# Nobita421/signature-Gan

Measured on AMD Instinct MI355X. Metric: signature images/sec (G+D train step, bs64 64x64 z=100), higher is better.
Workload: dtype f32; 1 GPU; configs[1]: reference conv G/D 64x64x1, z=100, batch 64 per GPU, f32, n_critic=1; global_batch=64, parallelism=dp1

## Files before the change

### include/siggan.h

```cpp
#ifndef SIGGAN_H
#define SIGGAN_H

#include <stddef.h>
#include <stdint.h>

#ifdef __cplusplus
extern "C" {
#endif

#define SIGGAN_ABI_VERSION 4

enum {
    SIGGAN_OK = 0,
    SIGGAN_E_INVALID = -1,
    SIGGAN_E_STATE = -2,
    SIGGAN_E_HIP = -3,
    SIGGAN_E_NOMEM = -4
};

typedef struct siggan_ctx siggan_ctx;

typedef struct siggan_config {
    int32_t device;
    int32_t latent_dim;
    int32_t image_size;
    int32_t image_channels;
    int32_t max_batch;
    float   dropout;
    float   leaky_slope;
    uint64_t seed;
    int32_t dtype;
    float   f16_grad_scale;
    int32_t spectral_norm;
    float   g_leaky_slope;
} siggan_config;
enum { SIGGAN_DTYPE_F32 = 0, SIGGAN_DTYPE_BF16 = 1, SIGGAN_DTYPE_F16 = 2 };

typedef struct siggan_storage {
    float *g_params, *g_grads, *g_exp_avg, *g_exp_avg_sq, *g_adam_steps;
    float *g_bn_running_mean, *g_bn_running_var;
    int64_t *g_bn_batches;
    float *d_params, *d_grads, *d_exp_avg, *d_exp_avg_sq, *d_adam_steps;
    float *d_sn_u, *d_sn_v;
} siggan_storage;

typedef struct siggan_hyper {
    double lr, beta1, beta2, eps;
    float label_smoothing;
    float clip_max_norm;
    float grad_scale;
} siggan_hyper;

enum {
    SIGGAN_M_D_LOSS = 0, SIGGAN_M_D_LOSS_REAL, SIGGAN_M_D_LOSS_FAKE, SIGGAN_M_D_REAL_MEAN,
    SIGGAN_M_D_FAKE_MEAN, SIGGAN_M_D_REAL_ACC, SIGGAN_M_D_FAKE_ACC, SIGGAN_M_D_GRAD_NORM,
    SIGGAN_M_G_LOSS, SIGGAN_M_G_FAKE_MEAN, SIGGAN_M_G_GRAD_NORM,
    SIGGAN_M_D_SKIPPED, SIGGAN_M_G_SKIPPED,
    SIGGAN_M_COUNT = 16
};

int siggan_abi_version(void);
const char *siggan_last_error(void);
int siggan_create(const siggan_config *cfg, siggan_ctx **out);
int siggan_destroy(siggan_ctx *ctx);

int64_t siggan_param_count(const siggan_ctx *ctx, int which);
int32_t siggan_param_tensors(const siggan_ctx *ctx, int which);
int siggan_param_span(const siggan_ctx *ctx, int which, int32_t idx, int64_t *offset, int64_t *numel);
int64_t siggan_bn_count(const siggan_ctx *ctx);
int64_t siggan_sn_count(const siggan_ctx *ctx, int which);
int32_t siggan_bn_layers(const siggan_ctx *ctx);
int64_t siggan_workspace_bytes(const siggan_ctx *ctx);

int siggan_bind(siggan_ctx *ctx, const siggan_storage *st);
int siggan_params_changed(siggan_ctx *ctx);
int siggan_seed(siggan_ctx *ctx, uint64_t seed, uint64_t offset);
int siggan_rng_state(siggan_ctx *ctx, uint64_t *seed, uint64_t *offset);
#define SIGGAN_MODE_GRAPH 1
#define SIGGAN_MODE_OVERLAP 2
int siggan_set_mode(siggan_ctx *ctx, int32_t mode);

enum { SIGGAN_STEP_TRAINER = 0, SIGGAN_STEP_ABLATION = 1 };
int siggan_set_step_variant(siggan_ctx *ctx, int32_t variant);

int siggan_g_forward(siggan_ctx *ctx, const float *z_dev, int32_t batch, int32_t training,
                     float *images_dev, void *stream);

enum { SIGGAN_IS_NEG = 0, SIGGAN_IS_INK_SIGNED = 1, SIGGAN_IS_INK_UNIT = 2, SIGGAN_IS_COUNT = 3 };
int siggan_g_generate_u8(siggan_ctx *ctx, const float *z_dev, int32_t batch, uint8_t *u8_dev,
                         float *images_dev, int32_t *stats_dev, float threshold, void *stream);

int siggan_d_forward(siggan_ctx *ctx, const float *x_dev, int32_t batch, int32_t training,
                     const float *masks_dev, float *probs_dev, float *features_dev, void *stream);

int siggan_d_step(siggan_ctx *ctx, const float *real_dev, int32_t batch, const float *z_dev,
                  const float *masks_dev, const siggan_hyper *hp, float *metrics_dev,
                  float *metrics_host, void *stream);
int siggan_g_step(siggan_ctx *ctx, int32_t batch, const float *z_dev, const siggan_hyper *hp,
                  float *metrics_dev, float *metrics_host, void *stream);

#define SIGGAN_COMM_ID_BYTES 128
int siggan_comm_unique_id(void *id_out);
int siggan_comm_init(siggan_ctx *ctx, int32_t rank, int32_t world, const void *id);
int siggan_comm_destroy(siggan_ctx *ctx);
int32_t siggan_comm_world(const siggan_ctx *ctx);
int siggan_comm_broadcast(siggan_ctx *ctx, void *buf_dev, int64_t bytes, int32_t root, void *stream);

int siggan_d_grads(siggan_ctx *ctx, const float *real_dev, int32_t batch, const float *z_dev,
                   const float *masks_dev, const siggan_hyper *hp, float *metrics_dev, void *stream);
int siggan_step_begin(siggan_ctx *ctx, const float *real_dev, int32_t batch, const float *z_dev,
                      const float *masks_dev, const float *zg_dev, const siggan_hyper *hp,
                      float *metrics_dev, void *stream);
int siggan_stage_real(siggan_ctx *ctx, const float *real_dev, int32_t batch, void *stream);
int siggan_d_apply(siggan_ctx *ctx, const siggan_hyper *hp, float *metrics_dev, float *metrics_host,
                   void *stream);
int siggan_g_grads(siggan_ctx *ctx, int32_t batch, const float *z_dev, const siggan_hyper *hp,
                   float *metrics_dev, void *stream);
int siggan_g_apply(siggan_ctx *ctx, const siggan_hyper *hp, float *metrics_dev, float *metrics_host,
                   void *stream);

int siggan_op_conv4x4s2(siggan_ctx *ctx, int32_t form, const void *in_dev, const float *w_dev,
                        void *out_dev, int32_t batch, int32_t h_in, int32_t c_in, int32_t c_out,
                        void *stream);
int siggan_op_conv4x4s2_wgrad(siggan_ctx *ctx, const void *small_dev, const void *large_dev,
                              float *dw_dev, int32_t batch, int32_t h_small, int32_t c_small,
                              int32_t c_large, void *stream);
int siggan_op_adam(siggan_ctx *ctx, float *p_dev, float *g_dev, float *m_dev, float *v_dev,
                   int64_t n, int32_t step, const siggan_hyper *hp, void *stream);
int siggan_op_randn(siggan_ctx *ctx, float *out_dev, int64_t n, void *stream);
int siggan_augment_batch(int32_t device, const uint8_t *cache_dev, int64_t n_images, const int32_t *index_dev,
                         const int32_t *params_dev, const int16_t *tables_dev, const float *lut_dev,
                         float *out_dev, int32_t batch, int32_t size, int32_t augment, int32_t fill,
                         void *stream);
int siggan_image_stats(int32_t device, const float *x_dev, int32_t batch, int64_t pixels,
                       float threshold, int32_t *stats_dev, void *stream);
int siggan_device_info(int32_t device, int32_t *compute_units, int32_t *clock_khz, int64_t *hbm_bytes);
int siggan_prof_enable(siggan_ctx *ctx, int32_t on);
int32_t siggan_prof_slots(void);
int siggan_prof_read(siggan_ctx *ctx, int32_t idx, char *name, int32_t name_cap, int64_t *launches,
                     double *ms, double *flops, double *bytes);
int siggan_prof_launch(siggan_ctx *ctx, int64_t idx, int32_t *fields, int32_t n, int64_t *count);

int siggan_debug_tensor(siggan_ctx *ctx, const char *name, int32_t index, float *out_dev, int64_t n, void *stream);

#ifdef __cplusplus
}
#endif
#endif
```

### signature-gan_amd/csrc/gconv.h

```cpp
#pragma once
#include <hip/hip_runtime.h>
#include <stdint.h>
#include <vector>

#include "act.h"

namespace siggan {

enum Epilogue : int {
    EPI_RAW = 0,
    EPI_BIAS_LRELU_DROP,
    EPI_AFFINE_RELU,
    EPI_LRELU_BWD,
    EPI_BN_BWD_STATS,
};

struct GConvArgs {
    int dt;
    const void* in;
    const void* wp;
    void* out;
    int B, Hi, Wi, Ci, Co;
    int lgHr, lgWr;
    int Ho, Wo;
    int form;
    int M;
    int epi;
    const float* bias;
    const float* noise;
    const float* scale;
    const float* shift;
    const void* aref;
    const float* bnp;
    float* stat0;
    float* stat1;
    int64_t stat_cap;
    const float* cls_w;
    float* cls_part;
    float slope;
    float gslope;
    float* slab;
    int64_t slab_floats;
    size_t slab_stride;
    const float* zeros;
};

struct BnBwdParams { f32x4 sc, sf, mu, rs; };
__device__ __forceinline__ BnBwdParams bn_bwd_params(const float* __restrict__ bnp, int Co, int co) {
    BnBwdParams q;
    q.sc = *reinterpret_cast<const f32x4*>(bnp + co); q.sf = *reinterpret_cast<const f32x4*>(bnp + Co + co);
    q.mu = *reinterpret_cast<const f32x4*>(bnp + 2 * Co + co); q.rs = *reinterpret_cast<const f32x4*>(bnp + 3 * Co + co);
    return q;
}
template <class T, bool LK>
__device__ __forceinline__ void bn_bwd_stat_terms(const f32x4 v, const f32x4 y, const BnBwdParams& q, float gs, f32x4& s0, f32x4& s1) {
#pragma unroll
    for (int e = 0; e < 4; ++e) {
        const float vq = (float)(T)v[e];
        const float d = g_dact<LK>(fmaf(y[e], q.sc[e], q.sf[e]), vq, gs);
        s0[e] += d;
        s1[e] = fmaf(d, (y[e] - q.mu[e]) * q.rs[e], s1[e]);
    }
}
__host__ __device__ inline bool gen_lk(const GConvArgs& a) {
    return a.gslope != 0.f && (a.epi == EPI_AFFINE_RELU || a.epi == EPI_BN_BWD_STATS);
}

struct WgradArgs {
    int dt;
    const void* S;
    const void* L;
    float* slab;
    float* dw;
    float* db;
    int B, Cs, Cl;
    int lgHs, lgWs, lgCl;
    int K;
    int kchunk;
    const float* zeros;
};

struct Prof {
    struct Rec {
        int id; double flops, bytes; hipEvent_t e0, e1;
        int form, epi_req, epi, M, Ci, Co;
    };
    static constexpr int NID = 8;
    std::vector<Rec> recs;
    static const char* name(int id);
    void begin(int id, double flops, double bytes, hipStream_t st);
    void shape(const GConvArgs& a, int epi_req);
    void clear();
};
extern Prof* g_prof;

int launch_gconv(const GConvArgs& a, hipStream_t st);
void launch_gconv16(int cfg, const GConvArgs& a, dim3 grid, hipStream_t st, hipEvent_t e0, hipEvent_t e1, int kq = 1);
void launch_wgrad16(bool small, const WgradArgs& a, dim3 grid, hipStream_t st, hipEvent_t e0, hipEvent_t e1);
int launch_wgrad(WgradArgs a, int max_splits, hipStream_t st);

}
```

### signature-gan_amd/csrc/gconv.hip

```cpp
#include "gconv.h"
#include <hip/hip_ext.h>

namespace siggan {


static constexpr int BK = 32;
static constexpr int PAD = 4;

__device__ __forceinline__ int xcd_remap(int bid, int nwg) {
    const int q = nwg >> 3, r = nwg & 7, xcd = bid & 7, idx = bid >> 3;
    return (xcd < r ? xcd * (q + 1) : r * (q + 1) + (xcd - r) * q) + idx;
}

template <int BM, int BN, int WM, int WN, int BK = 32, int DEEP = 0, int KQ = 1, bool LK = false>
__global__ __launch_bounds__(256 * KQ) void k_gconv(const GConvArgs a) {
    constexpr int TM = BM / (32 * WM), TN = BN / (32 * WN);
    constexpr int PA = BM / 32, PB = BN / 32;
    constexpr int KC = BK / 32;
    constexpr int LD = BK + 4;
    __shared__ __attribute__((aligned(16))) float smem[KQ * 2 * LD * (BM + BN)];
    const int quad = KQ > 1 ? (int)(threadIdx.x >> 8) : 0;
    float* const sA = smem + quad * (2 * LD * (BM + BN));
    float* const sB = sA + 2 * LD * BM;

    const int tid = threadIdx.x & 255, lane = tid & 63, wave = tid >> 6;
    const int li = lane & 31, lh = lane >> 5;
    const int wm = wave / WN, wn = wave % WN;
    const float* const a_in = static_cast<const float*>(a.in);
    const float* const a_wp = static_cast<const float*>(a.wp);

    const int tiles_n = a.Co / BN;
    const int bid = xcd_remap(blockIdx.x, gridDim.x);
    const int m0 = (bid / tiles_n) * BM, n0 = (bid % tiles_n) * BN;
    const int cls = blockIdx.z, ph = cls >> 1, pw = cls & 1;
    const int Hr = 1 << a.lgHr, Wr = 1 << a.lgWr;
    const int ntaps = a.form == 0 ? 16 : 4;
    const int Ktot = ntaps * a.Ci;
    const int lgcpt = 31 - __builtin_clz(a.Ci / BK);
    const int nk_all = ntaps << lgcpt;
    const int kper = (nk_all + gridDim.y * KQ - 1) / (gridDim.y * KQ);
    const int k_lo = (blockIdx.y * KQ + quad) * kper;
    const int k_hi = min(nk_all, k_lo + kper);
    const int nk = k_hi - k_lo;

    const int kc = tid & 7, rloc = tid >> 3;
    const float* a_base[PA];
    int a_ih0[PA], a_iw0[PA];
#pragma unroll
    for (int p = 0; p < PA; ++p) {
        const int m = m0 + rloc + 32 * p;
        if (m < a.M) {
            const int n = m >> (a.lgHr + a.lgWr);
            const int rh = (m >> a.lgWr) & (Hr - 1), rw = m & (Wr - 1);
            a_base[p] = a_in + (size_t)n * a.Hi * a.Wi * a.Ci + kc * 4;
            if (a.form == 0) { a_ih0[p] = 2 * rh - 1; a_iw0[p] = 2 * rw - 1; }
            else             { a_ih0[p] = rh + ph;    a_iw0[p] = rw + pw; }
        } else {
            a_base[p] = a_in; a_ih0[p] = -(1 << 20); a_iw0[p] = -(1 << 20);
        }
    }
    const float* wcur = a_wp + ((size_t)cls * a.Co + n0 + rloc) * Ktot + kc * 4 + (size_t)k_lo * BK;

    const float* a_cur[PA];
    int a_step[PA];
    int l_tap = k_lo >> lgcpt, l_cc = k_lo & ((1 << lgcpt) - 1);
    auto set_tap = [&]() __attribute__((always_inline)) {
        int dh, dw;
        if (a.form == 0) { dh = l_tap >> 2; dw = l_tap & 3; } else { dh = -(l_tap >> 1); dw = -(l_tap & 1); }
#pragma unroll
        for (int p = 0; p < PA; ++p) {
            const int ih = a_ih0[p] + dh, iw = a_iw0[p] + dw;
            const bool ok = (unsigned)ih < (unsigned)a.Hi && (unsigned)iw < (unsigned)a.Wi;
            a_cur[p] = ok ? a_base[p] + ((size_t)(ih * a.Wi + iw) * a.Ci + l_cc * BK) : a.zeros;
            a_step[p] = ok ? BK : 0;
        }
    };
    constexpr int NSET = DEEP ? 2 : 1;
    f32x4 ra[NSET][PA][KC], rb[NSET][PB][KC];
    auto load_tile = [&](int set = 0) __attribute__((always_inline)) {
#pragma unroll
        for (int p = 0; p < PA; ++p) {
#pragma unroll
            for (int q = 0; q < KC; ++q) ra[set][p][q] = *reinterpret_cast<const f32x4*>(a_cur[p] + 32 * q);
// ... 269 lines not shown
        for (int t = 0; t < 4; ++t)
            rb[t] = *reinterpret_cast<const f32x4*>(w_row + (size_t)cls * a.Co * Ktot + t * CI + cc * BK);
        ++l_k;
    };
    auto store_tile = [&](int buf) __attribute__((always_inline)) {
#pragma unroll
        for (int t = 0; t < 4; ++t)
            *reinterpret_cast<f32x4*>(sB + ((buf * 4 + t) * BN + rloc) * LD + kc * 4) = rb[t];
    };

    f32x16 acc[4];
#pragma unroll
    for (int cls = 0; cls < 4; ++cls)
#pragma unroll
        for (int r = 0; r < 16; ++r) acc[cls][r] = 0.f;

    load_tile();
    store_tile(0);
    load_tile();
    __syncthreads();

    const int ml = wave * 32 + li;
    const float* const pP = sP + (((ml >> a.lgWr) + 1) * Wp + (ml & (Wr - 1)) + 1) * LP + 4 * lh;

#pragma unroll
    for (int cls = 0; cls < 4; ++cls) {
        const int ph = cls >> 1, pw = cls & 1;
        for (int cc = 0; cc < NCC; ++cc) {
            const int kt = cls * NCC + cc, buf = kt & 1;
            const float* pA[4];
#pragma unroll
            for (int t = 0; t < 4; ++t) pA[t] = pP + ((ph - (t >> 1)) * Wp + (pw - (t & 1))) * LP + cc * BK;
            const float* pB = sB + (buf * 4 * BN + li) * LD + 4 * lh;
            f32x4 fa[2][4], fb[2][4];
#pragma unroll
            for (int t = 0; t < 4; ++t) {
                fa[0][t] = *reinterpret_cast<const f32x4*>(pA[t]);
                fb[0][t] = *reinterpret_cast<const f32x4*>(pB + t * BN * LD);
            }
#pragma unroll
            for (int c = 0; c < BK / 8; ++c) {
                const int cur = c & 1, nxt = cur ^ 1;
                if (c + 1 < BK / 8) {
#pragma unroll
                    for (int t = 0; t < 4; ++t) {
                        fa[nxt][t] = *reinterpret_cast<const f32x4*>(pA[t] + 8 * (c + 1));
                        fb[nxt][t] = *reinterpret_cast<const f32x4*>(pB + t * BN * LD + 8 * (c + 1));
                    }
                }
                __builtin_amdgcn_sched_barrier(0);
#pragma unroll
                for (int t = 0; t < 4; ++t)
#pragma unroll
                    for (int u = 0; u < 4; ++u)
                        acc[cls] = __builtin_amdgcn_mfma_f32_32x32x2f32(fa[cur][t][u], fb[cur][t][u], acc[cls], 0, 0, 0);
                if (c == 0 && kt + 1 < 4 * NCC) store_tile(buf ^ 1);
                if (c == 1 && kt + 2 < 4 * NCC) load_tile();
            }
            __syncthreads();
        }
    }

    const float sc = a.epi == EPI_AFFINE_RELU ? a.scale[li] : 1.f, sf = a.epi == EPI_AFFINE_RELU ? a.shift[li] : 0.f;
    const int Wo = 2 * Wr;
    float* const so = smem;
#pragma unroll
    for (int r = 0; r < 16; ++r) {
        const int mr = wave * 32 + (r & 3) + 8 * (r >> 2) + 4 * lh;
        const int rl = mr >> a.lgWr, rw = mr & (Wr - 1);
#pragma unroll
        for (int cls = 0; cls < 4; ++cls) {
            float v = acc[cls][r];
            if (a.epi == EPI_AFFINE_RELU) v = g_act<LK>(fmaf(v, sc, sf), a.gslope);
            so[(((2 * rl + (cls >> 1)) * Wo) + 2 * rw + (cls & 1)) * BN + li] = v;
        }
    }
    __syncthreads();
    f32x4* const dst = reinterpret_cast<f32x4*>(static_cast<float*>(a.out) + ((size_t)n_img * a.Ho + 2 * rh0) * a.Wo * BN);
    const f32x4* const src = reinterpret_cast<const f32x4*>(so);
#pragma unroll
    for (int q = 0; q < (BM * 4 * BN / 4) / 256; ++q) dst[q * 256 + tid] = src[q * 256 + tid];
}

template <class T, bool LK>
__global__ __launch_bounds__(256) void k_splitk_epilogue(const GConvArgs a, int nsplit, int64_t total4) {
    const int64_t i = (int64_t)blockIdx.x * 256 + threadIdx.x;
    if (a.epi == EPI_BN_BWD_STATS) {
        __shared__ __attribute__((aligned(16))) float sh[256 * 8];
        const int C4 = a.Co / 4, c4 = threadIdx.x & (C4 - 1);
        f32x4 s0 = {0.f, 0.f, 0.f, 0.f}, s1 = s0;
        if (i < total4) {
            const f32x4* sl = reinterpret_cast<const f32x4*>(a.slab);
            const size_t stride4 = a.slab_stride / 4;
            f32x4 v = sl[i];
            for (int z = 1; z < nsplit; ++z) v += sl[(size_t)z * stride4 + i];
            bn_bwd_stat_terms<T, LK>(v, ld4<T>(static_cast<const T*>(a.aref) + i * 4), bn_bwd_params(a.bnp, a.Co, c4 * 4), a.gslope, s0, s1);
            st4<T>(static_cast<T*>(a.out) + i * 4, v);
        }
        *reinterpret_cast<f32x4*>(sh + threadIdx.x * 8) = s0;
        *reinterpret_cast<f32x4*>(sh + threadIdx.x * 8 + 4) = s1;
        __syncthreads();
        if ((int)threadIdx.x < C4) {
            for (int k = 1; k < 256 / C4; ++k) {
                s0 += *reinterpret_cast<const f32x4*>(sh + (k * C4 + c4) * 8);
                s1 += *reinterpret_cast<const f32x4*>(sh + (k * C4 + c4) * 8 + 4);
            }
            *reinterpret_cast<f32x4*>(a.stat0 + (size_t)blockIdx.x * a.Co + c4 * 4) = s0;
            *reinterpret_cast<f32x4*>(a.stat1 + (size_t)blockIdx.x * a.Co + c4 * 4) = s1;
        }
        return;
    }
    if (i >= total4) return;
    const float4* sl = reinterpret_cast<const float4*>(a.slab);
    const size_t stride4 = a.slab_stride / 4;
    float4 v = sl[i];
    for (int z = 1; z < nsplit; ++z) {
        const float4 w = sl[(size_t)z * stride4 + i];
        v.x += w.x; v.y += w.y; v.z += w.z; v.w += w.w;
    }
    const int C4 = a.Co / 4;
    const int64_t per_img = (int64_t)C4 * a.Ho * a.Wo;
    const bool p2 = (C4 & (C4 - 1)) == 0 && (per_img & (per_img - 1)) == 0;
    const int c = (p2 ? (int)(i & (C4 - 1)) : (int)(i % C4)) * 4;
    const int64_t n = p2 ? i >> (63 - __builtin_clzll(per_img)) : i / per_img;
    float* e = reinterpret_cast<float*>(&v);
    if (a.epi == EPI_BIAS_LRELU_DROP) {
#pragma unroll
        for (int k = 0; k < 4; ++k) {
            float x = e[k] + a.bias[c + k];
            x = x > 0.f ? x : x * a.slope;
            if (a.noise) x *= a.noise[n * a.Co + c + k];
            e[k] = x;
        }
    } else if (a.epi == EPI_AFFINE_RELU) {
#pragma unroll
        for (int k = 0; k < 4; ++k) e[k] = g_act<LK>(fmaf(e[k], a.scale[c + k], a.shift[c + k]), a.gslope);
    } else if (a.epi == EPI_LRELU_BWD) {
        const f32x4 ar = ld4<T>(static_cast<const T*>(a.aref) + i * 4);
        const float* r = reinterpret_cast<const float*>(&ar);
#pragma unroll
        for (int k = 0; k < 4; ++k) {
            float x = e[k] * (r[k] > 0.f ? 1.f : a.slope);
            if (a.noise) x *= a.noise[n * a.Co + c + k];
            e[k] = x;
        }
    }
    st4<T>(static_cast<T*>(a.out) + i * 4, f32x4{v.x, v.y, v.z, v.w});
    if (a.cls_w) {
        __shared__ float shc[4];
        const f32x4 w4 = *reinterpret_cast<const f32x4*>(a.cls_w + (size_t)(p2 ? (i & (per_img - 1)) : (i % per_img)) * 4);
        float d = (float)(T)v.x * w4[0];
        d = fmaf((float)(T)v.y, w4[1], d); d = fmaf((float)(T)v.z, w4[2], d); d = fmaf((float)(T)v.w, w4[3], d);
#pragma unroll
        for (int o = 32; o > 0; o >>= 1) d += __shfl_down(d, o, 64);
        if ((threadIdx.x & 63) == 0) shc[threadIdx.x >> 6] = d;
        __syncthreads();
        if (threadIdx.x == 0) a.cls_part[blockIdx.x] = ((shc[0] + shc[1]) + shc[2]) + shc[3];
    }
}

Prof* g_prof = nullptr;

const char* Prof::name(int id) {
    static const char* n[NID] = {"k_gconv<128,128>", "k_gconv<128,64>", "k_gconv<64,64>", "k_gconv<128,32>",
                                 "k_wgrad<64,64>", "k_gconv_up4", "k_wgrad<32,128>", "?"};
    return n[id < 0 || id >= NID ? NID - 1 : id];
}
void Prof::begin(int id, double flops, double bytes, hipStream_t) {
    Rec r; r.id = id; r.flops = flops; r.bytes = bytes;
    r.form = r.epi_req = r.epi = r.M = r.Ci = r.Co = -1;
    (void)hipEventCreate(&r.e0); (void)hipEventCreate(&r.e1);
    recs.push_back(r);
}
void Prof::shape(const GConvArgs& a, int epi_req) {
    Rec& r = recs.back();
    r.form = a.form; r.epi_req = epi_req; r.epi = a.epi; r.M = a.M; r.Ci = a.Ci; r.Co = a.Co;
}
void Prof::clear() {
    for (auto& r : recs) { (void)hipEventDestroy(r.e0); (void)hipEventDestroy(r.e1); }
    recs.clear();
}

static double gconv_bytes(const GConvArgs& a) {
    const double es = (double)dt_size(a.dt);
    const double in = (double)a.B * a.Hi * a.Wi * a.Ci, out = (double)a.B * a.Ho * a.Wo * a.Co, w = 16.0 * a.Ci * a.Co;
    return es * (in + w + out * (a.epi == EPI_LRELU_BWD ? 2.0 : 1.0));
}
static double wgrad_bytes(const WgradArgs& a) {
    const double es = (double)dt_size(a.dt);
    return es * ((double)a.K * a.Cs + 4.0 * a.K * a.Cl) + 4.0 * 16.0 * a.Cs * a.Cl;
}

template <int BM, int BN, int WM, int WN, int BKT = 32, int DEEP = 0, int KQ = 1>
static int launch_cfg(const GConvArgs& a_in, hipStream_t st, int id, int nsplit) {
    GConvArgs a = a_in;
    const int tiles = ((a.M + BM - 1) / BM) * (a.Co / BN);
    const int ncls = a.form == 0 ? 1 : 4;
    const int64_t total4 = (int64_t)a.B * a.Ho * a.Wo * a.Co / 4;
    int rows = 0;
    if (a.epi == EPI_BN_BWD_STATS) {
        if (nsplit > 1 && (256 % (a.Co / 4)) != 0) nsplit = 1;
        rows = nsplit > 1 ? (int)((total4 + 255) / 256) : ((a.M + BM - 1) / BM) * ncls;
        if ((int64_t)2 * rows * a.Co > a.stat_cap) { a.epi = EPI_RAW; rows = 0; }
        else a.stat1 = a.stat0 + (size_t)rows * a.Co;
    }
    if (a.cls_w) {
        const int64_t per_img4 = (int64_t)a.Ho * a.Wo * a.Co / 4;
        if (nsplit > 1 && a.epi != EPI_BN_BWD_STATS && total4 % 256 == 0 && per_img4 % 256 == 0) rows = (int)(per_img4 / 256);
        else a.cls_w = nullptr;
    }
    dim3 grid(tiles, nsplit, ncls);
    if (g_prof) {
        g_prof->begin(id, 2.0 * a.M * a.Co * (double)((a.form == 0 ? 16 : 4) * a.Ci) * ncls, gconv_bytes(a), st);
        g_prof->shape(a, a_in.epi);
    }
    hipEvent_t e0 = g_prof ? g_prof->recs.back().e0 : nullptr, e1 = g_prof ? g_prof->recs.back().e1 : nullptr;
    if (a.dt != DT_F32) {
        launch_gconv16(id, a, grid, st, e0, e1, KQ);
    } else if (gen_lk(a)) {
        hipExtLaunchKernelGGL((k_gconv<BM, BN, WM, WN, BKT, DEEP, KQ, true>), grid, dim3(256 * KQ), 0, st, e0, e1, 0, a);
    } else if (g_prof) {
        hipExtLaunchKernelGGL((k_gconv<BM, BN, WM, WN, BKT, DEEP, KQ>), grid, dim3(256 * KQ), 0, st, e0, e1, 0, a);
    } else {
        hipLaunchKernelGGL((k_gconv<BM, BN, WM, WN, BKT, DEEP, KQ>), grid, dim3(256 * KQ), 0, st, a);
    }
    if (nsplit > 1)
        SIGGAN_GS_SWITCH(gen_lk(a) ? 1.f : 0.f, LK, SIGGAN_DT_SWITCH(a.dt, T, hipLaunchKernelGGL((k_splitk_epilogue<T, LK>),
            dim3((unsigned)((total4 + 255) / 256)), dim3(256), 0, st, a, nsplit, total4)));
    return rows;
}

int launch_gconv(const GConvArgs& a_in, hipStream_t st) {
    GConvArgs a = a_in;
    if (a.epi == EPI_BN_BWD_STATS && (a.stat0 == nullptr || a.stat_cap <= 0)) return -1;
    const int ncls = a.form == 0 ? 1 : 4;
    auto blocks = [&](int bm, int bn) { return ((a.M + bm - 1) / bm) * (a.Co / bn) * ncls; };
    const int nk = (a.form == 0 ? 16 : 4) * (a.Ci / BK);
    auto splits = [&](int nblk) {
        int ns = 1;
        if (a.slab && nblk < 384) {
            ns = (512 + nblk - 1) / nblk;
            if (ns > nk / 4) ns = nk / 4;
            if (ns > 8) ns = 8;
            const int64_t out_floats = (int64_t)a.B * a.Ho * a.Wo * a.Co;
            if (ns > 1 && (int64_t)ns * out_floats > a.slab_floats) ns = (int)(a.slab_floats / out_floats);
            if (ns < 1) ns = 1;
        }
        a.slab_stride = (size_t)a.B * a.Ho * a.Wo * a.Co;
        return ns;
    };
    if (a.Co >= 64) {
        if (a.Co >= 128 && blocks(128, 128) >= 512) return launch_cfg<128, 128, 2, 2, 32, 1>(a, st, 0, 1);
        const int ns = splits(blocks(64, 64));
        if (ns == 2 && (nk & 1) == 0) return launch_cfg<64, 64, 2, 2, 32, 1, 2>(a, st, 2, 1);
        if (ns == 4 && !a.cls_w && a.dt != DT_F32 && (nk & 1) == 0) return launch_cfg<64, 64, 2, 2, 32, 1, 2>(a, st, 2, 1);
        return launch_cfg<64, 64, 2, 2, 32, 1>(a, st, 2, ns);
    }
    if (a.dt == DT_F32 && a.form == 1 && a.Co == 32 && (a.epi == EPI_RAW || a.epi == EPI_AFFINE_RELU) && (a.Ci == 32 || a.Ci == 64) &&
        a.M / 128 >= (a.Ci == 32 ? 384 : 768) && a.M % 128 == 0 &&
        ((1 << (a.lgHr + a.lgWr)) % 128) == 0 && a.lgWr >= 4 && a.lgWr <= 6) {
        dim3 grid(a.M / 128);
        if (g_prof) {
            g_prof->begin(5, 2.0 * a.M * a.Co * (double)(4 * a.Ci) * 4, gconv_bytes(a), st);
            g_prof->shape(a, a.epi);
        }
        hipEvent_t e0 = g_prof ? g_prof->recs.back().e0 : nullptr, e1 = g_prof ? g_prof->recs.back().e1 : nullptr;
        if (gen_lk(a)) {
            if (a.Ci == 32) hipExtLaunchKernelGGL((k_gconv_up4<32, true>), grid, dim3(256), 0, st, e0, e1, 0, a);
            else hipExtLaunchKernelGGL((k_gconv_up4<64, true>), grid, dim3(256), 0, st, e0, e1, 0, a);
        } else {
            if (a.Ci == 32) hipExtLaunchKernelGGL((k_gconv_up4<32, false>), grid, dim3(256), 0, st, e0, e1, 0, a);
            else hipExtLaunchKernelGGL((k_gconv_up4<64, false>), grid, dim3(256), 0, st, e0, e1, 0, a);
        }
        return 0;
    }
    const int ns = splits(blocks(128, 32));
    return launch_cfg<128, 32, 4, 1, 32, 1>(a, st, 3, ns);
}

template <int BM, int BN, int WM, int WN>
__global__ __launch_bounds__(256) void k_wgrad(const WgradArgs a) {
    constexpr int TM = BM / (32 * WM), TN = BN / (32 * WN);
    constexpr int LDA = BM + PAD, LDB = BN + PAD;
    constexpr int CA = BM / 4, RA = 256 / CA, PA = BK / RA;
    constexpr int CB = BN / 4, RB = 256 / CB, PB = BK / RB;
    __shared__ __attribute__((aligned(16))) float smem[2 * BK * (LDA + LDB)];
    float* const sA = smem;
    float* const sB = smem + 2 * BK * LDA;

    const int tid = threadIdx.x, lane = tid & 63, wave = tid >> 6;
    const int li = lane & 31, lh = lane >> 5;
    const int wm = wave / WN, wn = wave % WN;
    const int N = 16 << a.lgCl;
    const int tiles_n = N / BN;
    const int lin = blockIdx.z * gridDim.x + blockIdx.x;
    const int lid = xcd_remap(lin, gridDim.x * gridDim.z);
    const int bx = lid % gridDim.x, bz = lid / gridDim.x;
    const int i0 = (bx / tiles_n) * BM, j0 = (bx % tiles_n) * BN;
    const int kbeg = bz * a.kchunk;
    const int kend = min(a.K, kbeg + a.kchunk);
    const int nk = (kend - kbeg + BK - 1) / BK;
    const int Hs = 1 << a.lgHs, Ws = 1 << a.lgWs, Hl = 2 * Hs, Wl = 2 * Ws, Cl = 1 << a.lgCl;

    const int ca = tid % CA, ka = tid / CA;
    const int cb = tid % CB, kb = tid / CB;
    const float* const a_S = static_cast<const float*>(a.S);
    const float* const a_L = static_cast<const float*>(a.L);
    const int jj = j0 + cb * 4, tap = jj >> a.lgCl, lch = jj & (Cl - 1);
    const int kh = tap >> 2, kw = tap & 3;

    f32x4 ra[2][PA], rb[2][PB];
    size_t a_off[PA];
    int a_pix[PA], b_pix[PB];
#pragma unroll
    for (int p = 0; p < PA; ++p) { a_pix[p] = kbeg + ka + RA * p; a_off[p] = (size_t)a_pix[p] * a.Cs + i0 + ca * 4; }
#pragma unroll
    for (int p = 0; p < PB; ++p) b_pix[p] = kbeg + kb + RB * p;
    const int a_adv = BK * a.Cs;
    const int lgWl = a.lgWs + 1;
#define WG_LOAD_TILE(KT, SET)                                                                         \
    {                                                                                                 \
        _Pragma("unroll") for (int p = 0; p < PA; ++p) {                                              \
            const float* src = a_pix[p] < kend ? a_S + a_off[p] : a.zeros;                            \
            ra[SET][p] = *reinterpret_cast<const f32x4*>(src);                                       \
            a_off[p] += a_adv; a_pix[p] += BK;                                                        \
        }                                                                                             \
        _Pragma("unroll") for (int p = 0; p < PB; ++p) {                                              \
            const int pix = b_pix[p];                                                                 \
            const int y = pix >> a.lgWs;                                              \
            const int ih = 2 * (y & (Hs - 1)) - 1 + kh, iw = 2 * (pix & (Ws - 1)) - 1 + kw;           \
            const bool ok = pix < kend && (unsigned)ih < (unsigned)Hl && (unsigned)iw < (unsigned)Wl; \
                          \
            const unsigned off = (((unsigned)(2 * y - 1 + kh) << lgWl) + (unsigned)iw) << a.lgCl;     \
            const float* src = ok ? a_L + ((size_t)off + lch) : a.zeros;                              \
            rb[SET][p] = *reinterpret_cast<const f32x4*>(src);                                       \
            b_pix[p] += BK;                                                                           \
        }                                                                                             \
    }
#define WG_STORE_TILE(BUF, SET)                                                                       \
    {                                                                                                 \
        _Pragma("unroll") for (int p = 0; p < PA; ++p)                                                \
            *reinterpret_cast<f32x4*>(sA + (BUF) * BK * LDA + (ka + RA * p) * LDA + ca * 4) = ra[SET][p]; \
        _Pragma("unroll") for (int p = 0; p < PB; ++p)                                                \
            *reinterpret_cast<f32x4*>(sB + (BUF) * BK * LDB + (kb + RB * p) * LDB + cb * 4) = rb[SET][p]; \
    }

    f32x16 acc[TM][TN];
#pragma unroll
    for (int i = 0; i < TM; ++i)
#pragma unroll
        for (int j = 0; j < TN; ++j)
#pragma unroll
            for (int r = 0; r < 16; ++r) acc[i][j][r] = 0.f;

    constexpr int NQ = 256 / BM, KQ = BK / NQ;
    const bool bias_blk = a.db != nullptr && j0 == 0;
    const int bcol = tid % BM, kq = tid / BM;
    float bsum = 0.f;
#define WG_TILE(BUF, ST, LD)                                                                          \
    {                                                                                                 \
// ... 171 lines not shown
```

### signature-gan_amd/csrc/ops.h

```cpp
#pragma once
#include <hip/hip_runtime.h>
#include <stdint.h>

#include "act.h"

namespace siggan {

struct DevState {
    unsigned long long seed;
    unsigned long long rng_ctr;
    float step_size;
    float bc2_sqrt;
    float grad_mul;
    float grad_norm;
    float sumsq;
    int skip;
    float pad[2];
};

void launch_randn(float* out, int64_t n, const DevState* st, uint32_t stream_id, hipStream_t s);
void launch_dropnoise_multi(int nt, float* const* out, const int64_t* n, const int64_t* elem0, const uint32_t* sid, float keep,
                            const DevState* st, hipStream_t s, uint32_t ctr_add = 0);
void launch_mask_to_noise(const float* mask, float* out, int64_t n, float keep, hipStream_t s);
void launch_tick(DevState* st, hipStream_t s);

enum PrepType : int { PREP_PACK_DOWN = 0, PREP_PACK_UP, PREP_FC_T, PREP_CLS, PREP_BN_EVAL, PREP_SCALE, PREP_TAPS };
struct PrepJob {
    int type, O, I, perm;
    int dt;
    const float* mul;
    const float* src;
    const float* src2;
    const float* src3;
    const float* src4;
    float* dst;
};
struct PrepTable {
    static constexpr int MAXJ = 32;
    int njobs;
    int overflow;
    long long prefix[MAXJ + 1];
    PrepJob job[MAXJ];
};
void prep_add(PrepTable& t, const PrepJob& j, long long count);
bool launch_prepare(const PrepTable& t, float bn_eps, hipStream_t s);
bool launch_prepare_conv1(const PrepTable& t, float bn_eps, int dt, const float* x, const float* W, const float* b, float slope,
                          void* out, int B, int S, hipStream_t s);

void launch_fc_fwd(int dt, const float* z, const float* Wt, const float* b, void* y, int B, int K, int C0, float gslope,
                   hipStream_t s, const float* bn_affine_relu = nullptr, const DevState* st = nullptr, uint32_t stream_id = 0,
                   float* z_out = nullptr);
bool launch_fc_fwd_fused(int dt, const float* z, const float* W, const float* bias, void* y, void* a, const float* gamma,
                         const float* beta, float* rmean, float* rvar, int64_t* batches, float* bn, const float* bne,
                         float* z_out, const DevState* st, uint32_t sid, int B, int K, int C0, float momentum, float eps,
                         float gslope, hipStream_t s);
bool launch_fc_bwd_fused(int dt, const void* da, const void* y, const float* z, float* bn, float* dW, float* db, float* dgamma,
                         float* dbeta, int B, int K, int C0, float gslope, hipStream_t s);
void launch_fc_wgrad(int dt, const void* dy, const float* z, float* dW, float* db, int B, int K, int C0, hipStream_t s);

void launch_bn_train_stats(int dt, const void* y, int64_t R, int C, const float* gamma, const float* beta,
                           float* rmean, float* rvar, int64_t* batches, float* bn, float* partial,
                           int perm_c0, float momentum, float eps, hipStream_t s);
void launch_bn_relu(int dt, const void* y, void* a, int64_t R, int C, const float* bn, float gslope, hipStream_t s);
void launch_bn_bwd(int dt, void* da, const void* y, int64_t R, int C, float* bn, float* partial,
                   float* dgamma, float* dbeta, int perm_c0, float gslope, hipStream_t s, int pre_rows = 0, hipEvent_t done = nullptr);

void launch_final_fwd(int dt, const void* act, const float* Wt, const float* b, float* img, int B, int S, int C, float gslope,
                      hipStream_t s, const float* bn = nullptr, hipEvent_t done = nullptr, uint8_t* u8 = nullptr,
                      int32_t* stats = nullptr, float thr = 0.f);
void launch_final_bwd_reduce(int dt, const float* dpre, const float* Wt, const void* y, int B, int S, int C, const float* bn,
                             float* partial, float* partial_w, float gslope, hipStream_t s);
void launch_final_bn_bwd_apply(int dt, const float* dpre, const float* Wt, const void* y, void* dy, int B, int S, int C, float* bn,
                               const float* partial, const float* partial_w, float* dW, float* db, float* dgamma, float* dbeta,
                               float gslope, hipStream_t s, hipEvent_t done = nullptr);

void launch_conv1_fwd(int dt, const float* x0, int n0, const float* x1, const float* W, const float* b,
                      const float* noise, float slope, void* out, int B, int S, int C, hipStream_t s);
void launch_conv1_wgrad(int dt, const void* dv, const float* x0, int n0, const float* x1, float* dW, float* db,
                        float* partial, int B, int S, int C, hipStream_t s);
void launch_conv1_dgrad_tanh(int dt, const void* dv, const float* Wt, const float* img, float* dpre, int B, int S,
                             int C, hipStream_t s);
void launch_cls_fwd(int dt, const void* act, const float* wcp, const float* bc, float* logits, int B, int F, hipStream_t s);
void launch_cls_features(int dt, const void* act, float* feat, int B, int C, hipStream_t s);
void launch_bce(const float* logits, int B, int n0, float y0, float y1, float* probs, float* dlogit,
                float* metrics, int is_g_step, hipStream_t s, float gscale = 1.0f, const float* parts = nullptr, int P = 0,
                const float* bc = nullptr);
void launch_cls_bwd(int dt, const float* logits, int n0, float y0, float y1, const float* wcp, const void* act, const float* noise,
                    float slope, void* dv, int B, int C, hipStream_t s, float gscale = 1.0f, float* bce_probs = nullptr,
                    float* bce_dlogit = nullptr, float* bce_metrics = nullptr, int bce_is_g = 0, bool with_bce = false,
                    const float* parts = nullptr, int P = 0, const float* bc = nullptr);
void launch_cls_wgrad(int dt, const float* dlogit, const void* act, float* dWc, float* dbc, int B, int C, hipStream_t s);
void launch_to_f32(int dt, const void* src, float* dst, int64_t n, hipStream_t s);

struct SnLayer {
    const float* W;
    int rows, K;
    int u_off, v_off;
    int64_t w_off;
};
struct SnTable {
    static constexpr int MAXS = 8;
    int n;
    SnLayer layer[MAXS];
    int pre_k[MAXS + 1], pre_r[MAXS + 1];
    float *u, *v;
    float *tbuf, *wbuf;
    float* sig;
    float *u_saved, *v_saved;
    float* dots;
    int u_total, v_total;
    int slot[2];
};
void launch_sn_sigma(const SnTable& t, int training, int slot, float eps, hipStream_t s);
void launch_sn_combine(const SnTable& t, const float* g0, const float* g1, float* out, int64_t total, int npass, hipStream_t s);

void launch_grad_sumsq(const float* g, int64_t n, DevState* st, float* partial, hipStream_t s);
void launch_adam_prepare(DevState* st, float* steps, int ntensors, double lr, double beta1, double beta2,
                         float grad_scale, float clip_max_norm, float* metric_norm, hipStream_t s,
                         int check_finite = 0, float* metric_skipped = nullptr, const float* sumsq_partial = nullptr);
__host__ __device__ inline double pow_step(double b, double t) {
    unsigned long long n = (unsigned long long)t;
    double r = 1.0;
    while (n) { if (n & 1) r *= b; b *= b; n >>= 1; }
    return r;
}
void launch_adam_fused(float* p, float* g, float* m, float* v, int64_t n, DevState* st, float* steps, int ntensors, double t,
                       double lr, double beta1, double beta2, double eps, float grad_scale, float clip_max_norm,
                       float* metric_norm, const float* sumsq_partial, hipStream_t s, float* metric_skipped = nullptr);
void launch_adam(float* p, float* g, float* m, float* v, int64_t n, const DevState* st, double beta1,
                 double beta2, double eps, int write_back_grad, hipStream_t s);

enum ApType : int { AP_FLAT = 0, AP_CONV, AP_T16, AP_TAPS, AP_BN };
struct ApJob {
    int type;
    int A, Bc;
    int dt;
    long long off, n;
    long long off2, n2;
    float* dst;
    float* dst2;
    const float* rmean;
    const float* rvar;
    int wait;
};
struct ApTable {
    static constexpr int MAXJ = 24;
    int njobs, overflow;
    long long prefix[MAXJ + 1];
    ApJob job[MAXJ];
};
void ap_add(ApTable& t, const ApJob& j);
struct ApRide { const float* x; void* out; int B, S, dt; float slope; long long w_off, b_off; unsigned* counter; unsigned* late; };
bool launch_adam_pack(const ApTable& t, float* p, float* g, float* m, float* v, DevState* st, float* steps, int ntensors,
                      double tstep, double lr, double beta1, double beta2, double eps, float grad_scale, float clip_max_norm,
                      float* metric_norm, const float* sumsq_partial, float* metric_skipped, float bn_eps,
                      const ApRide* ride, hipStream_t s);

// ... 8 lines not shown
```

### signature-gan_amd/csrc/ops.hip

```cpp
#include "ops.h"
#include "../../include/siggan.h"
#include "rng.h"

namespace siggan {

static inline int cdiv(int64_t a, int64_t b) { return (int)((a + b - 1) / b); }

__device__ __forceinline__ uint4 draw(const DevState* st, uint64_t idx, uint32_t stream_id, uint32_t ctr_add = 0) {
    return draw_raw(st->seed, st->rng_ctr + ctr_add, idx, stream_id);
}

__global__ void k_randn(float* __restrict__ out, int64_t n, const DevState* __restrict__ st, uint32_t sid) {
    const int64_t t = (int64_t)blockIdx.x * blockDim.x + threadIdx.x;
    if (t * 4 >= n) return;
    const f32x4 v = normal4(draw(st, (uint64_t)t, sid));
    for (int j = 0; j < 4 && t * 4 + j < n; ++j) out[t * 4 + j] = v[j];
}
__global__ void k_mask_to_noise(const float* __restrict__ m, float* __restrict__ out, int64_t n, float inv) {
    const int64_t i = (int64_t)blockIdx.x * blockDim.x + threadIdx.x;
    if (i < n) out[i] = m[i] * inv;
}
__global__ void k_tick(DevState* st) { st->rng_ctr += 1; }

void launch_randn(float* out, int64_t n, const DevState* st, uint32_t sid, hipStream_t s) {
    hipLaunchKernelGGL(k_randn, dim3(cdiv((n + 3) / 4, 256)), dim3(256), 0, s, out, n, st, sid);
}
struct NoiseTable { float* out[8]; int64_t n[8]; int64_t elem0[8]; uint32_t sid[8]; int64_t pre[9]; int nt; };
__global__ void k_dropnoise_multi(const NoiseTable tb, float keep, float inv, const DevState* __restrict__ st, uint32_t ctr_add) {
    const int64_t g = (int64_t)blockIdx.x * blockDim.x + threadIdx.x;
    if (g >= tb.pre[tb.nt]) return;
    int t = 0;
    while (g >= tb.pre[t + 1]) ++t;
    const int64_t q = g - tb.pre[t];
    const uint4 r = draw(st, (uint64_t)(tb.elem0[t] / 4 + q), tb.sid[t], ctr_add);
    const uint32_t x[4] = {r.x, r.y, r.z, r.w};
    float* o = tb.out[t];
    for (int j = 0; j < 4 && q * 4 + j < tb.n[t]; ++j) o[q * 4 + j] = u01(x[j]) < keep ? inv : 0.f;
}
void launch_dropnoise_multi(int nt, float* const* out, const int64_t* n, const int64_t* elem0, const uint32_t* sid, float keep,
                            const DevState* st, hipStream_t s, uint32_t ctr_add) {
    NoiseTable tb; tb.nt = nt; tb.pre[0] = 0;
    for (int t = 0; t < nt; ++t) { tb.out[t] = out[t]; tb.n[t] = n[t]; tb.elem0[t] = elem0[t]; tb.sid[t] = sid[t]; tb.pre[t + 1] = tb.pre[t] + (n[t] + 3) / 4; }
    hipLaunchKernelGGL(k_dropnoise_multi, dim3(cdiv(tb.pre[nt], 256)), dim3(256), 0, s, tb, keep, 1.0f / keep, st, ctr_add);
}
void launch_mask_to_noise(const float* mask, float* out, int64_t n, float keep, hipStream_t s) {
    hipLaunchKernelGGL(k_mask_to_noise, dim3(cdiv(n, 256)), dim3(256), 0, s, mask, out, n, 1.0f / keep);
}
void launch_tick(DevState* st, hipStream_t s) { hipLaunchKernelGGL(k_tick, dim3(1), dim3(1), 0, s, st); }

__device__ __forceinline__ int perm16(int c, int perm_c0) { return perm_c0 > 0 ? (c % perm_c0) * 16 + c / perm_c0 : c; }

struct AdamK { float mul, ss, bc2, w1, beta2, w2, eps; };
__device__ __forceinline__ void adam_upd(const AdamK& k, float& pp, float& gg, float& mm, float& vv) {
    const float gr = gg * k.mul;
    gg = gr;
    mm = k.w1 < 0.5f ? mm + k.w1 * (gr - mm) : gr - (gr - mm) * (1.0f - k.w1);
    vv = vv * k.beta2 + k.w2 * gr * gr;
    const float denom = sqrtf(vv) / k.bc2 + k.eps;
    pp = pp + (k.ss * mm) / denom;
}

static long long prep_units(const PrepJob& j) {
    switch (j.type) {
        case PREP_PACK_DOWN: case PREP_CLS: return j.type == PREP_CLS ? 1 : j.O;
        case PREP_PACK_UP: return j.O;
        case PREP_FC_T: return (long long)(j.I * 16 / 64) * ((j.O + 127) / 128);
        case PREP_SCALE: return (j.O + 1023) / 1024;
        case PREP_TAPS: return (j.O * j.I + 255) / 256;
        default: return (j.O + 255) / 256;
    }
}
void prep_add(PrepTable& t, const PrepJob& j, long long ) {
    if (t.njobs >= PrepTable::MAXJ) { t.overflow = 1; return; }
    if (t.njobs == 0) t.prefix[0] = 0;
    t.job[t.njobs] = j;
    t.prefix[t.njobs + 1] = t.prefix[t.njobs] + prep_units(j);
    ++t.njobs;
}
__device__ __forceinline__ void put_w(const PrepJob& q, size_t idx, float v) {
    if (q.mul) v *= q.mul[0];
    if (q.dt == DT_F32) q.dst[idx] = v;
    else if (q.dt == DT_BF16) reinterpret_cast<bf16_t*>(q.dst)[idx] = (bf16_t)v;
    else reinterpret_cast<f16_t*>(q.dst)[idx] = (f16_t)v;
// ... 376 lines not shown
    for (; k + 14 <= K; k += 14) {
        float w[14];
#pragma unroll
        for (int u = 0; u < 14; ++u) w[u] = wp[(size_t)(k + u) * F];
#pragma unroll
        for (int u = 0; u < 14; ++u)
#pragma unroll
            for (int j = 0; j < 8; ++j) acc[j] = fmaf(sz[j * K + k + u], w[u], acc[j]);
    }
    for (; k < K; ++k) {
        const float w = wp[(size_t)k * F];
#pragma unroll
        for (int j = 0; j < 8; ++j) acc[j] = fmaf(sz[j * K + k], w, acc[j]);
    }
    const float bias = b[(fp % C0) * 16 + fp / C0];
    if (bn) {
        const float sc = bn[fp], sf = bn[F + fp];
#pragma unroll
        for (int j = 0; j < 8; ++j)
            if (nb + j < B) st1<T>(y + (size_t)(nb + j) * F + fp, g_act<LK>(fmaf(acc[j] + bias, sc, sf), gs));
        return;
    }
#pragma unroll
    for (int j = 0; j < 8; ++j)
        if (nb + j < B) st1<T>(y + (size_t)(nb + j) * F + fp, acc[j] + bias);
}
void launch_fc_fwd(int dt, const float* z, const float* Wt, const float* b, void* y, int B, int K, int C0, float gslope,
                   hipStream_t s, const float* bn_affine_relu, const DevState* st, uint32_t stream_id, float* z_out) {
    SIGGAN_GS_SWITCH(gslope, LK, SIGGAN_DT_SWITCH(dt, T, hipLaunchKernelGGL((k_fc_fwd<T, LK>), dim3(cdiv(C0 * 16, 256), cdiv(B, 8)), dim3(256),
                                                                     8 * K * sizeof(float), s, z, Wt, b, (T*)y, B, K, C0, bn_affine_relu,
                                                                     st, stream_id, z_out, gslope)));
}
static constexpr int FK = 8;
template <class T>
__global__ __launch_bounds__(256) void k_fc_wgrad(const T* __restrict__ dy, const float* __restrict__ z, float* __restrict__ dW,
                           float* __restrict__ db, int B, int K, int C0) {
    __shared__ float sz[64][FK];
    const int F = C0 * 16;
    const int fp = blockIdx.x * 256 + threadIdx.x, k0 = blockIdx.y * FK;
    float acc[FK], sb = 0.f;
#pragma unroll
    for (int u = 0; u < FK; ++u) acc[u] = 0.f;
    for (int n0 = 0; n0 < B; n0 += 64) {
        __syncthreads();
        for (int i = threadIdx.x; i < 64 * FK; i += 256) {
            const int n = n0 + i / FK, k = k0 + i % FK;
            sz[i / FK][i % FK] = (n < B && k < K) ? z[(size_t)n * K + k] : 0.f;
        }
        __syncthreads();
        if (fp < F) {
            const int nn = B - n0 < 64 ? B - n0 : 64;
            int n = 0;
            for (; n + 8 <= nn; n += 8) {
                float g[8];
#pragma unroll
                for (int v = 0; v < 8; ++v) g[v] = ld1<T>(dy + (size_t)(n0 + n + v) * F + fp);
#pragma unroll
                for (int v = 0; v < 8; ++v) {
                    sb += g[v];
#pragma unroll
                    for (int u = 0; u < FK; ++u) acc[u] = fmaf(g[v], sz[n + v][u], acc[u]);
                }
            }
            for (; n < nn; ++n) {
                const float g = ld1<T>(dy + (size_t)(n0 + n) * F + fp);
                sb += g;
#pragma unroll
                for (int u = 0; u < FK; ++u) acc[u] = fmaf(g, sz[n][u], acc[u]);
            }
        }
    }
    if (fp >= F) return;
    const int f = (fp % C0) * 16 + fp / C0;
#pragma unroll
    for (int u = 0; u < FK; ++u)
        if (k0 + u < K) dW[(size_t)f * K + k0 + u] = acc[u];
    if (blockIdx.y == 0) db[f] = sb;
}
void launch_fc_wgrad(int dt, const void* dy, const float* z, float* dW, float* db, int B, int K, int C0, hipStream_t s) {
    SIGGAN_DT_SWITCH(dt, T, hipLaunchKernelGGL(k_fc_wgrad<T>, dim3(cdiv(C0 * 16, 256), cdiv(K, FK)), dim3(256), 0, s, (const T*)dy, z, dW, db,
                                                B, K, C0));
}

typedef f32x4 f4v;
__device__ __forceinline__ f4v ldg4(const float* p) { return *reinterpret_cast<const f4v*>(p); }
__device__ __forceinline__ int clampi(int v, int hi) { return v < 0 ? 0 : (v > hi ? hi : v); }

struct StripId { int n, y0, x; };
template <int RY>
__device__ __forceinline__ StripId strip_of(int sid, int S, int xi) {
    const int nbx = S >> 5, nby = S / RY;
    StripId r;
    r.x = (sid % nbx) * 32 + xi; sid /= nbx;
    r.y0 = (sid % nby) * RY; r.n = sid / nby;
    return r;
}

template <class T, bool BN, bool LK>
__global__ __launch_bounds__(256) void k_final_fwd(const T* __restrict__ act, const float* __restrict__ Wt,
                                                   const float* __restrict__ b, float* __restrict__ img, int S,
                                                   const float* __restrict__ bn, float gs) {
    constexpr int RY = 4, C = 32;
    const int c4 = threadIdx.x & 7;
    const StripId t = strip_of<RY>(blockIdx.x, S, threadIdx.x >> 3);
    f4v w[9];
#pragma unroll
    for (int k = 0; k < 9; ++k) w[k] = ldg4(Wt + k * 32 + c4 * 4);
    const float bias = b[0];
    f4v sc = {1.f, 1.f, 1.f, 1.f}, sf = {0.f, 0.f, 0.f, 0.f};
    if (BN) { sc = ldg4(bn + c4 * 4); sf = ldg4(bn + C + c4 * 4); }
    const T* base = act + (size_t)t.n * S * S * C + c4 * 4;
    f4v v[RY + 2][3];
#pragma unroll
    for (int r = 0; r < RY + 2; ++r) {
        const int yy = t.y0 + r - 1, yc = clampi(yy, S - 1);
#pragma unroll
        for (int d = 0; d < 3; ++d) {
            const int xx = t.x + d - 1, xc = clampi(xx, S - 1);
            f4v q = ld4<T>(base + ((size_t)yc * S + xc) * C);
            if (BN) q = f4v{g_act<LK>(fmaf(q.x, sc.x, sf.x), gs), g_act<LK>(fmaf(q.y, sc.y, sf.y), gs),
                            g_act<LK>(fmaf(q.z, sc.z, sf.z), gs), g_act<LK>(fmaf(q.w, sc.w, sf.w), gs)};
            v[r][d] = (yy == yc && xx == xc) ? q : f4v{0.f, 0.f, 0.f, 0.f};
        }
    }
#pragma unroll
    for (int r = 0; r < RY; ++r) {
        float acc = 0.f;
#pragma unroll
        for (int kh = 0; kh < 3; ++kh)
#pragma unroll
            for (int kw = 0; kw < 3; ++kw) {
                const f4v a = v[r + kh][kw], ww = w[kh * 3 + kw];
                acc = fmaf(a.x, ww.x, acc); acc = fmaf(a.y, ww.y, acc); acc = fmaf(a.z, ww.z, acc); acc = fmaf(a.w, ww.w, acc);
            }
        acc += __shfl_xor(acc, 4, 8); acc += __shfl_xor(acc, 2, 8); acc += __shfl_xor(acc, 1, 8);
        if (c4 == 0) img[((size_t)t.n * S + t.y0 + r) * S + t.x] = tanhf(acc + bias);
    }
}
template <class T>
__global__ __launch_bounds__(256) void k_final_fwd_u8(const T* __restrict__ act, const float* __restrict__ Wt,
                                                      const float* __restrict__ b, float* __restrict__ img,
                                                      uint8_t* __restrict__ u8, int32_t* __restrict__ stats, float thr, int S) {
    constexpr int RY = 4, C = 32;
    __shared__ int sh[4][SIGGAN_IS_COUNT];
    const int c4 = threadIdx.x & 7;
    const StripId t = strip_of<RY>(blockIdx.x, S, threadIdx.x >> 3);
    f4v w[9];
#pragma unroll
    for (int k = 0; k < 9; ++k) w[k] = ldg4(Wt + k * 32 + c4 * 4);
    const float bias = b[0];
    const T* base = act + (size_t)t.n * S * S * C + c4 * 4;
    f4v v[RY + 2][3];
#pragma unroll
    for (int r = 0; r < RY + 2; ++r) {
        const int yy = t.y0 + r - 1, yc = clampi(yy, S - 1);
#pragma unroll
        for (int d = 0; d < 3; ++d) {
            const int xx = t.x + d - 1, xc = clampi(xx, S - 1);
            const f4v q = ld4<T>(base + ((size_t)yc * S + xc) * C);
            v[r][d] = (yy == yc && xx == xc) ? q : f4v{0.f, 0.f, 0.f, 0.f};
        }
    }
    uint32_t rows = 0;
    int n_neg = 0, n_sig = 0, n_uni = 0;
#pragma unroll
    for (int r = 0; r < RY; ++r) {
        float acc = 0.f;
#pragma unroll
        for (int kh = 0; kh < 3; ++kh)
#pragma unroll
            for (int kw = 0; kw < 3; ++kw) {
                const f4v a = v[r + kh][kw], ww = w[kh * 3 + kw];
                acc = fmaf(a.x, ww.x, acc); acc = fmaf(a.y, ww.y, acc); acc = fmaf(a.z, ww.z, acc); acc = fmaf(a.w, ww.w, acc);
            }
        acc += __shfl_xor(acc, 4, 8); acc += __shfl_xor(acc, 2, 8); acc += __shfl_xor(acc, 1, 8);
        const float tv = tanhf(acc + bias);
        if (img && c4 == 0) img[((size_t)t.n * S + t.y0 + r) * S + t.x] = tv;
        const float u = tv + 1.0f;
        const float q = fminf(fmaxf(u * 127.5f, 0.f), 255.f);
        rows |= (uint32_t)(int)q << (8 * r);
        if (stats) {
            n_neg += __popcll(__ballot(tv < 0.f));
            n_sig += __popcll(__ballot(u * 0.5f < thr));
            n_uni += __popcll(__ballot(tv < thr));
        }
    }
    const int j = (threadIdx.x >> 3) & 3, sft = 8 * j;
    uint32_t out = ((rows >> sft) & 255u) << sft;
#pragma unroll
    for (int k = 1; k < 4; ++k) out |= ((__shfl_xor(rows, 8 * k) >> sft) & 255u) << (8 * (j ^ k));
    if (c4 == 0) *reinterpret_cast<uint32_t*>(u8 + ((size_t)t.n * S + t.y0 + j) * S + (t.x & ~3)) = out;
    if (stats) {
        if ((threadIdx.x & 63) == 0) {
            int* cnt = sh[threadIdx.x >> 6];
            cnt[SIGGAN_IS_NEG] = n_neg >> 3; cnt[SIGGAN_IS_INK_SIGNED] = n_sig >> 3; cnt[SIGGAN_IS_INK_UNIT] = n_uni >> 3;
        }
        __syncthreads();
        if (threadIdx.x < SIGGAN_IS_COUNT) {
            const int k = threadIdx.x, sum = sh[0][k] + sh[1][k] + sh[2][k] + sh[3][k];
            if (sum) atomicAdd(stats + (size_t)t.n * SIGGAN_IS_COUNT + k, sum);
        }
    }
}
void launch_final_fwd(int dt, const void* act, const float* Wt, const float* b, float* img, int B, int S, int C, float gslope,
                      hipStream_t s, const float* bn, hipEvent_t done, uint8_t* u8, int32_t* stats, float thr) {
    (void)C;
    const dim3 grid(B * (S / 4) * (S / 32));
    if (u8) {
        if (stats) (void)hipMemsetAsync(stats, 0, (size_t)B * SIGGAN_IS_COUNT * sizeof(int32_t), s);
        SIGGAN_DT_SWITCH(dt, T, SIGGAN_LAUNCH_EV(done, (k_final_fwd_u8<T>), grid, dim3(256), 0, s, (const T*)act, Wt, b, img, u8, stats, thr, S));
        return;
    }
    SIGGAN_DT_SWITCH(dt, T, {
        if (bn && gslope != 0.f) SIGGAN_LAUNCH_EV(done, (k_final_fwd<T, true, true>), grid, dim3(256), 0, s, (const T*)act, Wt, b, img, S, bn, gslope);
        else if (bn) SIGGAN_LAUNCH_EV(done, (k_final_fwd<T, true, false>), grid, dim3(256), 0, s, (const T*)act, Wt, b, img, S, bn, gslope);
        else SIGGAN_LAUNCH_EV(done, (k_final_fwd<T, false, false>), grid, dim3(256), 0, s, (const T*)act, Wt, b, img, S, bn, gslope);
    });
}

template <int RY>
__device__ __forceinline__ float dpre_patch_elem(const float* __restrict__ dpre, int n, int y0, int xb, int S, int idx) {
    constexpr int PW = 34;
    const int r = idx / PW, k = idx - r * PW;
    const int yy = y0 + r - 1, xx = xb + k - 1, yc = clampi(yy, S - 1), xc = clampi(xx, S - 1);
    const float q = dpre[((size_t)n * S + yc) * S + xc];
    return (yy == yc && xx == xc && idx < (RY + 2) * PW) ? q : 0.f;
}
template <int RY>
__device__ __forceinline__ void read_dpre_patch(const float* sp, int xi, float (&d)[RY + 2][3]) {
#pragma unroll
    for (int r = 0; r < RY + 2; ++r)
#pragma unroll
        for (int k = 0; k < 3; ++k) d[r][k] = sp[r * 34 + xi + k];
}
template <int RY>
__device__ __forceinline__ f4v final_dact(const float (&d)[RY + 2][3], const f4v (&w)[9], int r) {
    f4v acc = {0.f, 0.f, 0.f, 0.f};
#pragma unroll
    for (int kh = 0; kh < 3; ++kh)
#pragma unroll
        for (int kw = 0; kw < 3; ++kw) {
            const float g = d[r + 2 - kh][2 - kw];
            const f4v ww = w[kh * 3 + kw];
            acc.x = fmaf(g, ww.x, acc.x); acc.y = fmaf(g, ww.y, acc.y); acc.z = fmaf(g, ww.z, acc.z); acc.w = fmaf(g, ww.w, acc.w);
        }
    return acc;
}

template <class T, int RY, bool LK>
__global__ __launch_bounds__(256) void k_final_bwd_reduce(const float* __restrict__ dpre, const float* __restrict__ Wt,
                                                          const T* __restrict__ y, const float* __restrict__ bn,
                                                          float* __restrict__ p0, float* __restrict__ p1,
                                                          float* __restrict__ pw, int S, int nstrips, float gs) {
    constexpr int C = 32;
    __shared__ f4v sh[2][4][8];
    __shared__ float shw[4][8][37];
    const int c4 = threadIdx.x & 7, wave = threadIdx.x >> 6;
    f4v w[9];
#pragma unroll
    for (int k = 0; k < 9; ++k) w[k] = ldg4(Wt + k * 32 + c4 * 4);
    const f4v sc = ldg4(bn + c4 * 4), sf = ldg4(bn + C + c4 * 4), mu = ldg4(bn + 2 * C + c4 * 4), rs = ldg4(bn + 3 * C + c4 * 4);
    f4v s0 = {0.f, 0.f, 0.f, 0.f}, s1 = s0;
    f4v acc[9];
#pragma unroll
    for (int k = 0; k < 9; ++k) acc[k] = f4v{0.f, 0.f, 0.f, 0.f};
    float sdb = 0.f;
    __shared__ float sp[2][(RY + 2) * 34];
    const int xi = threadIdx.x >> 3;
    f4v yn[RY];
    float pn;
    {
        const StripId t0 = strip_of<RY>(blockIdx.x < (unsigned)nstrips ? blockIdx.x : 0, S, xi);
        const T* yb = y + (((size_t)t0.n * S + t0.y0) * S + t0.x) * C + c4 * 4;
#pragma unroll
        for (int r = 0; r < RY; ++r) yn[r] = ld4<T>(yb + (size_t)r * S * C);
        pn = dpre_patch_elem<RY>(dpre, t0.n, t0.y0, t0.x - xi, S, threadIdx.x);
    }
    int it = 0;
    for (int sid = blockIdx.x; sid < nstrips; sid += gridDim.x, it ^= 1) {
        if (threadIdx.x < (RY + 2) * 34) sp[it][threadIdx.x] = pn;
        __syncthreads();
        f4v yv[RY];
#pragma unroll
        for (int r = 0; r < RY; ++r) yv[r] = yn[r];
        {
            const int nx = sid + gridDim.x < nstrips ? sid + gridDim.x : sid;
            const StripId tn = strip_of<RY>(nx, S, xi);
            const T* yb = y + (((size_t)tn.n * S + tn.y0) * S + tn.x) * C + c4 * 4;
#pragma unroll
            for (int r = 0; r < RY; ++r) yn[r] = ld4<T>(yb + (size_t)r * S * C);
            pn = dpre_patch_elem<RY>(dpre, tn.n, tn.y0, tn.x - xi, S, threadIdx.x);
        }
        float d[RY + 2][3];
        read_dpre_patch<RY>(sp[it], xi, d);
#pragma unroll
        for (int r = 0; r < RY; ++r) {
            const f4v g = final_dact<RY>(d, w, r);
            const f4v v = yv[r];
            const f4v pre = {fmaf(v.x, sc.x, sf.x), fmaf(v.y, sc.y, sf.y), fmaf(v.z, sc.z, sf.z), fmaf(v.w, sc.w, sf.w)};
            const f4v m = {g_dact<LK>(pre.x, g.x, gs), g_dact<LK>(pre.y, g.y, gs), g_dact<LK>(pre.z, g.z, gs), g_dact<LK>(pre.w, g.w, gs)};
            s0 += m;
            s1.x = fmaf(m.x, (v.x - mu.x) * rs.x, s1.x); s1.y = fmaf(m.y, (v.y - mu.y) * rs.y, s1.y);
            s1.z = fmaf(m.z, (v.z - mu.z) * rs.z, s1.z); s1.w = fmaf(m.w, (v.w - mu.w) * rs.w, s1.w);
            const f4v a = {g_act<LK>(pre.x, gs), g_act<LK>(pre.y, gs), g_act<LK>(pre.z, gs), g_act<LK>(pre.w, gs)};
            sdb += d[r + 1][1];
#pragma unroll
            for (int kh = 0; kh < 3; ++kh)
#pragma unroll
                for (int kw = 0; kw < 3; ++kw) {
                    const float gg = d[r + 2 - kh][2 - kw];
                    f4v& q = acc[kh * 3 + kw];
                    q.x = fmaf(a.x, gg, q.x); q.y = fmaf(a.y, gg, q.y); q.z = fmaf(a.z, gg, q.z); q.w = fmaf(a.w, gg, q.w);
                }
        }
    }
#pragma unroll
    for (int o = 8; o < 64; o <<= 1) {
        s0.x += __shfl_xor(s0.x, o); s0.y += __shfl_xor(s0.y, o); s0.z += __shfl_xor(s0.z, o); s0.w += __shfl_xor(s0.w, o);
        s1.x += __shfl_xor(s1.x, o); s1.y += __shfl_xor(s1.y, o); s1.z += __shfl_xor(s1.z, o); s1.w += __shfl_xor(s1.w, o);
#pragma unroll
        for (int k = 0; k < 9; ++k) {
            acc[k].x += __shfl_xor(acc[k].x, o); acc[k].y += __shfl_xor(acc[k].y, o);
            acc[k].z += __shfl_xor(acc[k].z, o); acc[k].w += __shfl_xor(acc[k].w, o);
        }
        sdb += __shfl_xor(sdb, o);
    }
    if ((threadIdx.x & 63) < 8) {
        sh[0][wave][c4] = s0; sh[1][wave][c4] = s1;
#pragma unroll
        for (int k = 0; k < 9; ++k) {
            shw[wave][c4][0 * 9 + k] = acc[k].x; shw[wave][c4][1 * 9 + k] = acc[k].y;
            shw[wave][c4][2 * 9 + k] = acc[k].z; shw[wave][c4][3 * 9 + k] = acc[k].w;
        }
        shw[wave][c4][36] = sdb;
    }
    __syncthreads();
    if (threadIdx.x < 8) {
        const f4v a = ((sh[0][0][c4] + sh[0][1][c4]) + sh[0][2][c4]) + sh[0][3][c4];
        const f4v b = ((sh[1][0][c4] + sh[1][1][c4]) + sh[1][2][c4]) + sh[1][3][c4];
        *reinterpret_cast<f4v*>(p0 + (size_t)blockIdx.x * C + c4 * 4) = a;
        *reinterpret_cast<f4v*>(p1 + (size_t)blockIdx.x * C + c4 * 4) = b;
    }
    float* out = pw + (size_t)blockIdx.x * (C * 9 + 1);
    for (int o = threadIdx.x; o < C * 9 + 1; o += 256) {
        const int g = o < C * 9 ? o / 36 : 0, j = o < C * 9 ? o % 36 : 36;
        out[o] = ((shw[0][g][j] + shw[1][g][j]) + shw[2][g][j]) + shw[3][g][j];
    }
}
template <class T, bool LK>
__global__ __launch_bounds__(256) void k_final_bnbwd_apply(const float* __restrict__ dpre, const float* __restrict__ Wt,
                                                           const T* __restrict__ y, const float* __restrict__ bn,
                                                           T* __restrict__ dy, int S, float gs) {
    constexpr int RY = 4, C = 32;
    const int c4 = threadIdx.x & 7;
    const StripId t = strip_of<RY>(blockIdx.x, S, threadIdx.x >> 3);
    f4v w[9];
#pragma unroll
    for (int k = 0; k < 9; ++k) w[k] = ldg4(Wt + k * 32 + c4 * 4);
    const f4v sc = ldg4(bn + c4 * 4), sf = ldg4(bn + C + c4 * 4), mu = ldg4(bn + 2 * C + c4 * 4), rs = ldg4(bn + 3 * C + c4 * 4);
    const f4v c1 = ldg4(bn + 4 * C + c4 * 4), c2 = ldg4(bn + 5 * C + c4 * 4);
    __shared__ float sp[(RY + 2) * 34];
    const int xi = threadIdx.x >> 3;
    const float pe = dpre_patch_elem<RY>(dpre, t.n, t.y0, t.x - xi, S, threadIdx.x);
    const size_t o0 = (((size_t)t.n * S + t.y0) * S + t.x) * C + c4 * 4;
    f4v yv[RY];
#pragma unroll
    for (int r = 0; r < RY; ++r) yv[r] = ld4<T>(y + o0 + (size_t)r * S * C);
    if (threadIdx.x < (RY + 2) * 34) sp[threadIdx.x] = pe;
    __syncthreads();
    float d[RY + 2][3];
    read_dpre_patch<RY>(sp, xi, d);
#pragma unroll
    for (int r = 0; r < RY; ++r) {
        const f4v g = final_dact<RY>(d, w, r);
        const f4v v = yv[r];
        f4v o;
        o.x = sc.x * (g_dact<LK>(fmaf(v.x, sc.x, sf.x), g.x, gs) - c1.x - (v.x - mu.x) * rs.x * c2.x);
        o.y = sc.y * (g_dact<LK>(fmaf(v.y, sc.y, sf.y), g.y, gs) - c1.y - (v.y - mu.y) * rs.y * c2.y);
        o.z = sc.z * (g_dact<LK>(fmaf(v.z, sc.z, sf.z), g.z, gs) - c1.z - (v.z - mu.z) * rs.z * c2.z);
        o.w = sc.w * (g_dact<LK>(fmaf(v.w, sc.w, sf.w), g.w, gs) - c1.w - (v.w - mu.w) * rs.w * c2.w);
        st4<T>(dy + o0 + (size_t)r * S * C, o);
    }
}
__global__ __launch_bounds__(1024) void k_rows_sum(const float* __restrict__ partial, int nch, int width, float* __restrict__ o0, int n0,
                           float* __restrict__ o1) {
    __shared__ float sh[2][16][64];
    float s, q;
    gather2(partial, nullptr, nch, width, s, q, sh);
    const int j = blockIdx.x * 64 + (threadIdx.x & 63);
    if (threadIdx.x >= 64 || j >= width) return;
    if (j < n0) o0[j] = s; else o1[j - n0] = s;
}
__global__ __launch_bounds__(1024) void k_final_fin(const float* __restrict__ partial_w, int nch_w, int width, float* __restrict__ dW,
                                                    int n0, float* __restrict__ db, int nbw, const float* __restrict__ p0,
                                                    const float* __restrict__ p1, int nch, int64_t R, int C, float* __restrict__ bn,
                                                    float* __restrict__ dgamma, float* __restrict__ dbeta) {
    __shared__ float sh[2][16][64];
    float s, q;
    if ((int)blockIdx.x < nbw) {
        gather2(partial_w, nullptr, nch_w, width, s, q, sh);
        const int j = blockIdx.x * 64 + (threadIdx.x & 63);
        if (threadIdx.x >= 64 || j >= width) return;
        if (j < n0) dW[j] = s; else db[j - n0] = s;
        return;
    }
    const int bx = blockIdx.x - nbw;
    gather2<32>(p0, p1, nch, C, s, q, sh, bx);
    const int c = bx * 32 + (threadIdx.x & 31);
    if (threadIdx.x >= 32 || c >= C) return;
    dbeta[c] = s; dgamma[c] = q;
    const float invR = 1.0f / (float)R;
    bn[4 * C + c] = s * invR; bn[5 * C + c] = q * invR;
}
constexpr int FINAL_RY = 4;
static int final_reduce_rows(int B, int S) {
    const int n = B * (S / FINAL_RY) * (S / 32); return n < 512 ? n : 512;
}
void launch_final_bwd_reduce(int dt, const float* dpre, const float* Wt, const void* y, int B, int S, int C, const float* bn,
                             float* partial, float* partial_w, float gslope, hipStream_t s) {
    const int nstrips = B * (S / FINAL_RY) * (S / 32), nch = final_reduce_rows(B, S);
    float* p0 = partial; float* p1 = partial + (size_t)nch * C;
    SIGGAN_GS_SWITCH(gslope, LK, SIGGAN_DT_SWITCH(dt, T, hipLaunchKernelGGL((k_final_bwd_reduce<T, FINAL_RY, LK>), dim3(nch), dim3(256), 0, s, dpre, Wt,
                                                                     (const T*)y, bn, p0, p1, partial_w, S, nstrips, gslope)));
}
void launch_final_bn_bwd_apply(int dt, const float* dpre, const float* Wt, const void* y, void* dy, int B, int S, int C, float* bn,
                               const float* partial, const float* partial_w, float* dW, float* db, float* dgamma, float* dbeta,
                               float gslope, hipStream_t s, hipEvent_t done) {
    const int nstrips = B * (S / 4) * (S / 32), nch = final_reduce_rows(B, S);
    const float* p0 = partial; const float* p1 = partial + (size_t)nch * C;
    const int nbw = cdiv(C * 9 + 1, 64);
    hipLaunchKernelGGL(k_final_fin, dim3(nbw + cdiv(C, 32)), dim3(1024), 0, s, partial_w, nch, C * 9 + 1, dW, C * 9, db, nbw, p0, p1, nch,
                       (int64_t)B * S * S, C, bn, dgamma, dbeta);
    SIGGAN_GS_SWITCH(gslope, LK, SIGGAN_DT_SWITCH(dt, T, SIGGAN_LAUNCH_EV(done, (k_final_bnbwd_apply<T, LK>), dim3(nstrips), dim3(256), 0, s, dpre, Wt,
                                                                   (const T*)y, bn, (T*)dy, S, gslope)));
}

__device__ __forceinline__ const float* seg_ptr(const float* x0, int n0, const float* x1, int n, int S) {
    return n < n0 ? x0 + (size_t)n * S * S : x1 + (size_t)(n - n0) * S * S;
}
template <int RY>
__device__ __forceinline__ void stage_x(float* sx, const float* xp, int oh0, int S) {
    const int Wp = S + 2;
    for (int i = threadIdx.x; i < (2 * RY + 2) * Wp; i += 256) {
        const int r = i / Wp, cc = i - r * Wp, ih = 2 * oh0 - 1 + r, iw = cc - 1;
        sx[i] = ((unsigned)ih < (unsigned)S && (unsigned)iw < (unsigned)S) ? xp[ih * S + iw] : 0.f;
    }
}

struct Conv1Ride { const float *pw, *gw, *mw, *vw, *pb, *gb, *mb, *vb; unsigned* counter; AdamK k; };
template <class T, bool RIDE = false>
__device__ __forceinline__ void conv1_fwd_block(const float* __restrict__ x0, int n0, const float* __restrict__ x1,
                                                const float* __restrict__ W, const float* __restrict__ b,
                                                const float* __restrict__ noise, float slope,
                                                T* __restrict__ out, int S, unsigned bid, const Conv1Ride* rd = nullptr) {
    constexpr int RY = 2, C = 64;
    __shared__ float sx[(2 * RY + 2) * 130];
    __shared__ __attribute__((aligned(16))) float sw[16 * (C + 4)];
    __shared__ __attribute__((aligned(16))) float sb[RIDE ? C : 4];
    const int Ho = S >> 1, nby = Ho / RY, Wp = S + 2;
    const int n = bid / nby, oh0 = (bid % nby) * RY;
    const int q = threadIdx.x & 15, pl = threadIdx.x >> 4;
    stage_x<RY>(sx, seg_ptr(x0, n0, x1, n, S), oh0, S);
    f4v bias;
    if (RIDE) {
        for (int i = threadIdx.x; i < 16 * C; i += 256) {
            float pp = rd->pw[i], gg = rd->gw[i], mm = rd->mw[i], vv = rd->vw[i];
            adam_upd(rd->k, pp, gg, mm, vv);
            sw[(i & 15) * (C + 4) + (i >> 4)] = pp;
        }
        if (threadIdx.x < C) {
            float pp = rd->pb[threadIdx.x], gg = rd->gb[threadIdx.x], mm = rd->mb[threadIdx.x], vv = rd->vb[threadIdx.x];
            adam_upd(rd->k, pp, gg, mm, vv);
            sb[threadIdx.x] = pp;
        }
    } else {
        for (int i = threadIdx.x; i < 16 * C; i += 256) sw[(i & 15) * (C + 4) + (i >> 4)] = W[i];
        bias = ldg4(b + q * 4);
    }
    f4v nz = {1.f, 1.f, 1.f, 1.f};
    if (noise) nz = ldg4(noise + (size_t)n * C + q * 4);
    __syncthreads();
    if (RIDE) {
        if (threadIdx.x == 0) __hip_atomic_fetch_add(rd->counter, 1u, __ATOMIC_RELAXED, __HIP_MEMORY_SCOPE_AGENT);
        bias = *reinterpret_cast<const f4v*>(sb + q * 4);
    }
    f4v w[16];
#pragma unroll
    for (int t = 0; t < 16; ++t) w[t] = *reinterpret_cast<const f4v*>(sw + t * (C + 4) + q * 4);
    for (int p = pl; p < RY * Ho; p += 16) {
        const int r = p / Ho, ow = p - r * Ho;
        const float* xr = sx + (2 * r) * Wp + 2 * ow;
        f4v acc = bias;
#pragma unroll
        for (int kh = 0; kh < 4; ++kh)
#pragma unroll
            for (int kw = 0; kw < 4; ++kw) {
                const float xv = xr[kh * Wp + kw];
                const f4v wv = w[kh * 4 + kw];
                acc.x = fmaf(xv, wv.x, acc.x); acc.y = fmaf(xv, wv.y, acc.y);
                acc.z = fmaf(xv, wv.z, acc.z); acc.w = fmaf(xv, wv.w, acc.w);
            }
        acc.x = acc.x > 0.f ? acc.x : acc.x * slope; acc.y = acc.y > 0.f ? acc.y : acc.y * slope;
        acc.z = acc.z > 0.f ? acc.z : acc.z * slope; acc.w = acc.w > 0.f ? acc.w : acc.w * slope;
        if (noise) { acc.x *= nz.x; acc.y *= nz.y; acc.z *= nz.z; acc.w *= nz.w; }
        st4<T>(out + (((size_t)n * Ho + oh0 + r) * Ho + ow) * C + q * 4, acc);
    }
}
template <class T>
__global__ __launch_bounds__(256) void k_conv1_fwd(const float* __restrict__ x0, int n0, const float* __restrict__ x1,
                                                   const float* __restrict__ W, const float* __restrict__ b,
                                                   const float* __restrict__ noise, float slope,
                                                   T* __restrict__ out, int S) {
    conv1_fwd_block<T>(x0, n0, x1, W, b, noise, slope, out, S, blockIdx.x);
}
template <class T>
// ... 724 lines not shown
```

### signature-gan_amd/csrc/siggan.hip

```cpp
#include <hip/hip_runtime.h>
#include <dlfcn.h>
#include <math.h>
#include <stdarg.h>
#include <stdio.h>
#include <stdlib.h>
#include <string.h>
#include <new>
#include <vector>

#include "../../include/siggan.h"
#include "gconv.h"
#include "ops.h"

using namespace siggan;

static thread_local char g_err[512] = "";
static int fail(int code, const char* fmt, ...) {
    va_list ap;
    va_start(ap, fmt);
    vsnprintf(g_err, sizeof g_err, fmt, ap);
    va_end(ap);
    return code;
}
int siggan_set_error(int code, const char* fmt, ...) {
// ... 253 lines not shown
    case INV_WEIGHTS: c->g_dirty = c->d_dirty = true; c->adam_t_known[0] = c->adam_t_known[1] = false; cs.early_ar = false; [[fallthrough]];
    case INV_ROWS:    cs.conv1_rode = 0;                                               [[fallthrough]];
    case INV_STREAM:  drop_dreal(c); break;
    case INV_COMM:    cs.early_ar = false; break;
    }
}

extern "C" int siggan_create(const siggan_config* cfg, siggan_ctx** out) {
    if (!cfg || !out) return fail(SIGGAN_E_INVALID, "null argument");
    if (cfg->image_size != 64 && cfg->image_size != 128)
        return fail(SIGGAN_E_INVALID, "output_size must be 64 or 128, got %d", cfg->image_size);
    if (cfg->image_channels != 1) return fail(SIGGAN_E_INVALID, "only image_channels == 1 is built, got %d", cfg->image_channels);
    if (cfg->latent_dim < 1 || cfg->latent_dim > 4096) return fail(SIGGAN_E_INVALID, "latent_dim out of range: %d", cfg->latent_dim);
    if (cfg->max_batch < 1 || cfg->max_batch > 4096) return fail(SIGGAN_E_INVALID, "max_batch out of range: %d", cfg->max_batch);
    if (!(cfg->dropout >= 0.f && cfg->dropout < 1.f)) return fail(SIGGAN_E_INVALID, "dropout must be in [0,1)");
    if (cfg->dtype != SIGGAN_DTYPE_F32 && cfg->dtype != SIGGAN_DTYPE_BF16 && cfg->dtype != SIGGAN_DTYPE_F16)
        return fail(SIGGAN_E_INVALID, "dtype must be SIGGAN_DTYPE_F32, _BF16 or _F16, got %d", cfg->dtype);
    if (!(cfg->f16_grad_scale >= 0.f) || cfg->f16_grad_scale > 65536.f)
        return fail(SIGGAN_E_INVALID, "f16_grad_scale must be in [0, 65536] (0 = default)");
    if (!(cfg->g_leaky_slope >= 0.f) || !isfinite(cfg->g_leaky_slope))
        return fail(SIGGAN_E_INVALID, "g_leaky_slope must be finite and >= 0 (0 = ReLU), got %g", (double)cfg->g_leaky_slope);
    DevGuard dg(cfg->device);
    HIPCHK(dg.err);
    siggan_ctx* c = new (std::nothrow) siggan_ctx();
    if (!c) return fail(SIGGAN_E_NOMEM, "out of host memory");
    c->cfg = *cfg; c->S = cfg->image_size; c->latent = cfg->latent_dim; c->Bm = cfg->max_batch;
    c->dt = cfg->dtype; c->es = dt_size(c->dt);
    c->fc_fused = cfg->max_batch <= 256 && (cfg->latent_dim & 3) == 0;
    c->variant = SIGGAN_STEP_TRAINER;
    c->sn = cfg->spectral_norm != 0;
    c->gscale = c->dt == DT_F16 ? (cfg->f16_grad_scale > 0.f ? cfg->f16_grad_scale : 1024.f) : 1.0f;
    c->bound = false;
    invalidate(c, INV_INIT);
    build_layout(c);

    const int64_t Bm = c->Bm, Bd = 2 * Bm;
    size_t off = 0;
    char* base = nullptr;
    auto carve = [&](float** p, int64_t nfloats) {
        if (base) *p = (float*)(base + off);
        off += ((size_t)nfloats * sizeof(float) + 255) & ~(size_t)255;
    };
    auto carve_t = [&](char** p, int64_t nelem) {
        if (base) *p = base + off;
        off += ((size_t)nelem * c->es + 255) & ~(size_t)255;
    };
    c->slab_floats = (int64_t)16 << 20;
    c->slab_k_floats = (int64_t)16 << 20;
    for (int pass = 0; pass < 2; ++pass) {
        off = 0;
        carve(&c->z, Bm * c->latent);
        carve_t(&c->fc_y, Bm * c->F);
        for (int l = 0; l <= c->Lg; ++l) {
            const int64_t H = 4 << l, n = Bm * H * H * c->gC[l];
            if (l == 0) c->g_y[0] = c->fc_y; else carve_t(&c->g_y[l], n);
            carve_t(&c->g_a[l], n);
            if (c->dt != DT_F32) carve_t(&c->g_ae[l], n); else if (pass == 1) c->g_ae[l] = c->g_a[l];
            carve_t(&c->g_da[l], n);
            carve(&c->g_bn[l], 6 * (int64_t)(l == 0 ? c->F : c->gC[l]));
            carve(&c->g_bne[l], 4 * (int64_t)(l == 0 ? c->F : c->gC[l]));
        }
        if (pass == 1) c->g_y[0] = c->fc_y;
        carve(&c->img, Bm * c->S * c->S);
        carve(&c->dpre, Bm * c->S * c->S);
        for (int l = 1; l <= c->Ld; ++l) {
            const int64_t H = c->S >> l, n = Bd * H * H * c->dC[l];
            carve_t(&c->d_a[l], n);
            carve_t(&c->d_dv[l], n);
            carve(&c->d_noise[l], Bd * c->dC[l]);
        }
        carve(&c->logits, Bd); carve(&c->probs, Bd); carve(&c->dlogit, Bd);
        carve(&c->lparts, (int64_t)Bd * 16);
        for (int l = 1; l <= c->Lg; ++l) {
            carve_t(&c->g_up[l], (int64_t)c->gC[l - 1] * c->gC[l] * 16);
            carve_t(&c->g_dn[l], (int64_t)c->gC[l - 1] * c->gC[l] * 16);
        }
        for (int l = 2; l <= c->Ld; ++l) {
            carve_t(&c->d_dn[l], (int64_t)c->dC[l - 1] * c->dC[l] * 16);
            carve_t(&c->d_up[l], (int64_t)c->dC[l - 1] * c->dC[l] * 16);
        }
        carve(&c->wcp, (int64_t)c->dC[c->Ld] * 16);
        carve(&c->slab, c->slab_floats);
        carve(&c->slab_k, c->slab_k_floats);
        if (c->dt != DT_F32) carve(&c->slab_b, c->slab_floats); else if (pass == 1) c->slab_b = c->slab;
        carve(&c->slab_k2, c->slab_k_floats);
        if (c->dt != DT_F32) carve(&c->slab_k3, c->slab_k_floats); else if (pass == 1) c->slab_k3 = c->slab_k2;
        carve(&c->partial, PARTIAL_FLOATS);
        carve(&c->partial_b, PARTIAL_FLOATS);
        carve(&c->partial_c, PARTIAL_FLOATS);
        carve(&c->z_g, Bm * c->latent);
        carve(&c->img_g, Bm * c->S * c->S);
        carve(&c->real_stage, Bm * c->S * c->S);
        { int64_t sumC = 0; for (int l = 1; l <= c->Ld; ++l) sumC += c->dC[l]; carve(&c->mask_stage, 3 * Bm * sumC); }
        if (c->sn) {
            int64_t ut = 1, vt = (int64_t)c->dC[c->Ld] * 16;
            for (int l = 1; l <= c->Ld; ++l) { ut += c->dC[l]; vt += (int64_t)c->dC[l - 1] * 16; }
            carve(&c->sn_tbuf, vt); carve(&c->sn_wbuf, ut);
            carve(&c->sn_sig, 3 * 2 * SnTable::MAXS);
            carve(&c->sn_us, 3 * ut); carve(&c->sn_vs, 3 * vt);
            carve(&c->sn_dots, 2 * SnTable::MAXS * 64);
            carve(&c->sn_g[0], c->d_total); carve(&c->sn_g[1], c->d_total);
            carve(&c->d_w1s, (int64_t)c->dC[1] * 16);
        }
        carve(&c->metrics, SIGGAN_M_COUNT);
        carve_t(&c->op_pack, (int64_t)512 * 512 * 16);
        carve(&c->zeros, 64);
        carve(&c->wfc_t, (int64_t)c->F * c->latent);
        carve(&c->wfin_t, (int64_t)9 * c->gC[c->Lg]);
        carve(&c->d_w1t, (int64_t)16 * c->dC[1]);
        carve(&c->ride_ctr, 64);
        float* devp = nullptr;
        carve(&devp, 64);
        if (pass == 1) c->dev = (DevState*)devp;
        if (pass == 0) {
            c->ws_bytes = off;
            hipError_t e = hipMalloc((void**)&base, off);
            if (e != hipSuccess) { delete c; return fail(SIGGAN_E_NOMEM, "hipMalloc(%zu) -> %s", off, hipGetErrorString(e)); }
            c->ws = base;
        }
    }
    HIPCHK(hipMemset(c->ws, 0, c->ws_bytes));
    DevState h; memset(&h, 0, sizeof h);
    h.seed = cfg->seed; h.rng_ctr = 0; h.grad_mul = 1.f;
    HIPCHK(hipMemcpy(c->dev, &h, sizeof h, hipMemcpyHostToDevice));
    c->mode = SIGGAN_MODE_OVERLAP;
    c->evi = 0;
    HIPCHK(hipStreamCreateWithFlags(&c->s_m, hipStreamNonBlocking));
    HIPCHK(hipStreamCreateWithFlags(&c->s_a, hipStreamNonBlocking));
    HIPCHK(hipStreamCreateWithFlags(&c->s_b, hipStreamNonBlocking));
    HIPCHK(hipStreamCreateWithFlags(&c->s_c, hipStreamNonBlocking));
    HIPCHK(hipStreamCreateWithFlags(&c->s_n, hipStreamNonBlocking));
    HIPCHK(hipEventCreateWithFlags(&c->ev_gfwd, EV_FLAGS));
    HIPCHK(hipEventCreateWithFlags(&c->ev_dreal, EV_FLAGS));
    HIPCHK(hipEventCreateWithFlags(&c->ev_ar, hipEventDisableTiming));
    for (int i = 0; i < 2; ++i) HIPCHK(hipEventCreateWithFlags(&c->ev_sys[i], hipEventDisableTiming));
    c->lane_err = hipSuccess;
    c->comm = nullptr; c->comm_rank = 0; c->comm_world = 1; c->comm_err = 0;
    HIPCHK(hipHostMalloc((void**)&c->ride_late, sizeof(unsigned), hipHostMallocCoherent | hipHostMallocMapped));
    *c->ride_late = 0u;
    HIPCHK(hipHostGetDevicePointer((void**)&c->ride_late_dev, c->ride_late, 0));
    for (int i = 0; i < siggan_ctx::NEV; ++i) HIPCHK(hipEventCreateWithFlags(&c->ev[i], EV_FLAGS));
    for (int i = 0; i < siggan_ctx::NEV; ++i) HIPCHK(hipEventCreateWithFlags(&c->ev_fenced[i], hipEventDisableTiming));
    for (int i = 0; i < 2; ++i) HIPCHK(hipEventCreateWithFlags(&c->ev_bridge[i], hipEventDisableTiming));
    *out = c;
    return SIGGAN_OK;
}

extern "C" int siggan_destroy(siggan_ctx* c) {
    if (!c) return SIGGAN_OK;
    DevGuard dg(c->cfg.device);
    (void)hipDeviceSynchronize();
    if (c->comm) { (void)rccl()->CommDestroy(c->comm); c->comm = nullptr; }
    for (auto& e : c->graphs) (void)hipGraphExecDestroy(e.exec);
    for (int i = 0; i < siggan_ctx::NEV; ++i) if (c->ev[i]) (void)hipEventDestroy(c->ev[i]);
    for (int i = 0; i < siggan_ctx::NEV; ++i) if (c->ev_fenced[i]) (void)hipEventDestroy(c->ev_fenced[i]);
    for (int i = 0; i < 2; ++i) if (c->ev_bridge[i]) (void)hipEventDestroy(c->ev_bridge[i]);
    if (c->s_m) (void)hipStreamDestroy(c->s_m);
    if (c->s_a) (void)hipStreamDestroy(c->s_a);
    if (c->s_b) (void)hipStreamDestroy(c->s_b);
    if (c->s_c) (void)hipStreamDestroy(c->s_c);
    if (c->s_n) (void)hipStreamDestroy(c->s_n);
    if (c->ev_ar) (void)hipEventDestroy(c->ev_ar);
    for (int i = 0; i < 2; ++i) if (c->ev_sys[i]) (void)hipEventDestroy(c->ev_sys[i]);
    if (c->ev_gfwd) (void)hipEventDestroy(c->ev_gfwd);
    if (c->ev_dreal) (void)hipEventDestroy(c->ev_dreal);
    if (c->ws) (void)hipFree(c->ws);
    if (c->ride_late) (void)hipHostFree(c->ride_late);
// ... 340 lines not shown
    if (P == 0)
        launch_cls_fwd(c->dt, act(c->Ld), c->wcp, DP(c, di_cls_b(c)), c->logits + r0, nB, c->dC[c->Ld] * 16, s);
    return P;
}

struct BceSpec { int n0; float y0, y1; float* mt; int is_g; };

static bool d_backward_pass(const siggan_ctx* c, Lanes& L, const float* x0, int n0, const float* x1, int Bd, bool dropout,
                            bool want_wgrad, bool want_dimage, const BceSpec& bce, int P, int r0 = 0, float* garena = nullptr,
                            bool early_allreduce = false) {
    bool early_ar = false;
    const float slope = c->cfg.leaky_slope;
    const int Ld = c->Ld;
    float* const ga = garena ? garena : c->st.d_grads;
    auto G_ = [&](int i) { return ga + c->d_off[i]; };
    auto act = [&](int l) { const int64_t H = c->S >> l; return c->d_a[l] + (size_t)((int64_t)r0 * H * H * c->dC[l]) * c->es; };
    auto dvp = [&](int l) { const int64_t H = c->S >> l; return c->d_dv[l] + (size_t)((int64_t)r0 * H * H * c->dC[l]) * c->es; };
    auto nz = [&](int l) { return dropout ? c->d_noise[l] + (int64_t)r0 * c->dC[l] : nullptr; };
    hipStream_t const sb = want_wgrad ? L.b : L.m;
    if (P < 0) { L.note(hipErrorInvalidValue); return false; }
    const float* const parts = P ? c->lparts + (size_t)r0 * P : nullptr;
    const float* const bc = DP(c, di_cls_b(c));
    if (sb != L.m) {
        L.fork(L.b);
        launch_bce(c->logits + r0, Bd, bce.n0, bce.y0, bce.y1, c->probs + r0, c->dlogit + r0, bce.mt, bce.is_g, sb, c->gscale, parts, P, bc);
    }
    launch_cls_bwd(c->dt, c->logits + r0, bce.n0, bce.y0, bce.y1, c->wcp, act(Ld), nz(Ld), slope, dvp(Ld), Bd,
                   c->dC[Ld], L.m, c->gscale, c->probs + r0, c->dlogit + r0, bce.mt, bce.is_g, sb == L.m, parts, P, bc);
    if (want_wgrad)
        launch_cls_wgrad(c->dt, c->dlogit + r0, act(Ld), G_(di_cls_w(c)), G_(di_cls_b(c)), Bd, c->dC[Ld], sb);
    for (int l = Ld; l >= 2; --l) {
        const int Ho = c->S >> l, Hi = 2 * Ho, Co = c->dC[l], Ci = c->dC[l - 1];
        const bool w_main = want_wgrad && l == 2 && c->dt != DT_F32 && garena == nullptr;
        auto wgrad_l = [&](hipStream_t st, float* slab) {
            WgradArgs w; memset(&w, 0, sizeof w); w.zeros = c->zeros; w.dt = c->dt;
            w.S = dvp(l); w.L = act(l - 1); w.slab = slab; w.dw = G_(di_w(l)); w.B = Bd; w.Cs = Co; w.Cl = Ci;
            w.lgHs = ilog2i(Ho); w.lgWs = w.lgHs; w.lgCl = ilog2i(Ci); w.K = Bd * Ho * Ho;
            w.db = G_(di_b(l));
            const int max_splits = (int)(c->slab_floats / ((int64_t)Co * (16 * Ci + 1)));
            launch_wgrad(w, max_splits, st);
        };
        if (want_wgrad && !w_main) {
            L.fork(L.a);
            wgrad_l(L.a, c->slab);
            if (early_allreduce && l == Ld && c->comm && !c->comm_err && garena == nullptr) {
                hipEvent_t ea = c->ev_sys[0], eb = c->ev_sys[1];
                L.record(ea, L.a); L.record(eb, sb);
                L.wait(c->s_n, ea); L.wait(c->s_n, eb);
                const int64_t o = c->d_off[di_w(l)];
                const int rc = rccl()->AllReduce(ga + o, ga + o, (size_t)(c->d_total - o), NCCL_FLOAT32, NCCL_SUM, c->comm, c->s_n);
                if (rc != NCCL_SUCCESS) L.comm_fail(rc);
                else { L.record(c->ev_ar, c->s_n); early_ar = true; }
            }
        }
        GConvArgs a = gconv_args(c);
        a.in = dvp(l); a.wp = c->d_up[l]; a.out = dvp(l - 1);
        a.B = Bd; a.Hi = Ho; a.Wi = Ho; a.Ci = Co; a.Co = Ci;
        a.lgHr = ilog2i(Ho); a.lgWr = a.lgHr; a.Ho = Hi; a.Wo = Hi; a.form = 1; a.M = Bd * Ho * Ho;
        a.epi = EPI_LRELU_BWD; a.aref = act(l - 1); a.noise = nz(l - 1); a.slope = slope;
        launch_gconv(a, L.m);
        if (w_main) {
            L.fork(L.b);
            launch_conv1_wgrad(c->dt, dvp(1), x0, n0, x1, G_(di_w(1)), G_(di_b(1)), c->partial_b, Bd, c->S, c->dC[1], L.b);
            wgrad_l(L.m, c->slab_b);
        }
    }
    if (want_wgrad && c->dt != DT_F32 && garena == nullptr) {
        L.join(L.a);
        L.join(L.b);
    } else if (want_wgrad) {
        launch_conv1_wgrad(c->dt, dvp(1), x0, n0, x1, G_(di_w(1)), G_(di_b(1)), c->partial_b, Bd, c->S, c->dC[1], L.m);
        L.join(L.b);
        if (L.tail_wait) L.wait(L.m, L.tail_wait);
        L.join(L.a);
    }
    if (want_dimage)
        launch_conv1_dgrad_tanh(c->dt, dvp(1), c->d_w1t, x0, c->dpre, Bd, c->S, c->dC[1], L.m);
    return early_ar;
}

static void g_backward_pass(const siggan_ctx* c, Lanes& L, const float* z, int B) {
    const float gs = c->cfg.g_leaky_slope;
    const int Lg = c->Lg, S = c->S;
    int pre_rows = 0;
    for (int l = Lg; l >= 1; --l) {
        const int Hi = 4 << (l - 1), Ho = 2 * Hi, Ci = c->gC[l - 1], Co = c->gC[l];
        const int64_t R = (int64_t)B * Ho * Ho;
        hipEvent_t const ef = L.fork_event(L.a);
        if (l == Lg) {
            launch_final_bwd_reduce(c->dt, c->dpre, c->wfin_t, c->g_y[l], B, S, Co, c->g_bn[l], c->partial, c->partial_b, gs, L.m);
            launch_final_bn_bwd_apply(c->dt, c->dpre, c->wfin_t, c->g_y[l], c->g_da[l], B, S, Co, c->g_bn[l], c->partial, c->partial_b,
                                      GG(c, gi_fin_w(c)), GG(c, gi_fin_b(c)), GG(c, gi_bn_w(l)), GG(c, gi_bn_b(l)), gs, L.m, ef);
        } else
            launch_bn_bwd(c->dt, c->g_da[l], c->g_y[l], R, Co, c->g_bn[l], c->partial, GG(c, gi_bn_w(l)), GG(c, gi_bn_b(l)), 0, gs, L.m, pre_rows, ef);
        L.fork_after(L.a, ef);
        WgradArgs w; memset(&w, 0, sizeof w); w.zeros = c->zeros; w.dt = c->dt;
        w.S = c->g_a[l - 1]; w.L = c->g_da[l]; w.slab = c->slab; w.dw = GG(c, gi_up_w(l)); w.B = B; w.Cs = Ci; w.Cl = Co;
        w.lgHs = ilog2i(Hi); w.lgWs = w.lgHs; w.lgCl = ilog2i(Co); w.K = B * Hi * Hi;
        const int max_splits = (int)(c->slab_floats / ((int64_t)Ci * (16 * Co + 1)));
        launch_wgrad(w, max_splits, L.a);
        GConvArgs a = gconv_args(c);
        a.in = c->g_da[l]; a.wp = c->g_dn[l]; a.out = c->g_da[l - 1];
        a.B = B; a.Hi = Ho; a.Wi = Ho; a.Ci = Co; a.Co = Ci;
        a.lgHr = ilog2i(Hi); a.lgWr = a.lgHr; a.Ho = Hi; a.Wo = Hi; a.form = 0; a.M = B * Hi * Hi; a.epi = EPI_RAW;
        if (l >= 2) {
            a.epi = EPI_BN_BWD_STATS; a.aref = c->g_y[l - 1]; a.bnp = c->g_bn[l - 1]; a.stat0 = c->partial; a.stat_cap = PARTIAL_FLOATS;
        }
        pre_rows = launch_gconv(a, L.m);
        if (pre_rows < 0) {
            L.refuse("the Generator's input-gradient GEMM was refused: its BatchNorm-backward sums had no carve (stat_cap)");
            pre_rows = 0;
        }
    }
    if (!(c->fc_fused && launch_fc_bwd_fused(c->dt, c->g_da[0], c->fc_y, z, c->g_bn[0], GG(c, gi_fc_w()), GG(c, gi_fc_b()),
                                             GG(c, gi_bn0_w()), GG(c, gi_bn0_b()), B, c->latent, c->gC[0], gs, L.m))) {
        launch_bn_bwd(c->dt, c->g_da[0], c->fc_y, B, c->F, c->g_bn[0], c->partial, GG(c, gi_bn0_w()), GG(c, gi_bn0_b()),
                      c->gC[0], gs, L.m);
        launch_fc_wgrad(c->dt, c->g_da[0], z, GG(c, gi_fc_w()), GG(c, gi_fc_b()), B, c->latent, c->gC[0], L.m);
    }
    L.join(L.a);
}

static void make_noise(const siggan_ctx* c, const float* masks, int B, int p0, int p1, hipStream_t s, uint32_t ctr_add = 0) {
    const float keep = 1.0f - c->cfg.dropout;
    int64_t sumC = 0;
    for (int l = 1; l <= c->Ld; ++l) sumC += c->dC[l];
    if (!masks) {
        float* out[8]; int64_t n[8], e0[8]; uint32_t sid[8];
        for (int l = 1; l <= c->Ld; ++l) {
            const int64_t nl = (int64_t)B * c->dC[l];
            out[l - 1] = c->d_noise[l] + p0 * nl; n[l - 1] = nl * (p1 - p0); e0[l - 1] = p0 * nl; sid[l - 1] = 16 + l;
        }
        launch_dropnoise_multi(c->Ld, out, n, e0, sid, keep, c->dev, s, ctr_add);
        return;
    }
    int64_t pre = 0;
    for (int l = 1; l <= c->Ld; ++l) {
        const int64_t n = (int64_t)B * c->dC[l];
        for (int p = p0; p < p1; ++p)
            launch_mask_to_noise(masks + (int64_t)p * B * sumC + (int64_t)B * pre, c->d_noise[l] + p * n, n, keep, s);
        pre += c->dC[l];
    }
}

static int check_hyper(const siggan_hyper* hp) {
    if (!hp) return fail(SIGGAN_E_INVALID, "null hyper-parameters");
    if (!(hp->lr >= 0.0) || !(hp->beta1 >= 0.0 && hp->beta1 < 1.0) || !(hp->beta2 >= 0.0 && hp->beta2 < 1.0) || !(hp->eps >= 0.0))
        return fail(SIGGAN_E_INVALID, "invalid Adam hyper-parameters");
    return SIGGAN_OK;
}

static const float SN_EPS = 1e-12f;

static void phase_d_grads_sn(const siggan_ctx* c, Lanes& L, const PhaseKey& k, PhaseResult& r) {
    const int B = k.B;
    const bool drop = c->cfg.dropout > 0.f;
    repack(c, L, L.m, L.m, k.g_dirty != 0, false);
    if (k.pre_real)
        L.note(hipMemcpyAsync(c->real_stage, k.staged_src, (size_t)B * c->S * c->S * sizeof(float), hipMemcpyDeviceToDevice, L.m));
    if (drop) make_noise(c, k.has_masks ? c->mask_stage : nullptr, B, 0, 2, L.m);
    const float* fake = c->img;
    if (k.variant == SIGGAN_STEP_ABLATION) {
        r.ga_last_B = g_forward_pass(c, k.has_zg ? c->z_g : nullptr, B, true, c->img_g, L.m, nullptr, nullptr, 2, c->z_g);
        L.record(c->ev_gfwd, L.m);
        fake = c->img_g;
    } else {
        r.ga_last_B = g_forward_pass(c, k.has_z ? c->z : nullptr, B, false, c->img, L.m, nullptr, nullptr, 1, c->z);
    }
    launch_sn_sigma(c->snt, 1, 0, SN_EPS, L.m);
    repack(c, L, L.m, L.m, false, true, 0);
    r.lP[0] = d_forward_rows(c, c->real_stage, 0, B, drop, L.m, c->slab_k);
    launch_sn_sigma(c->snt, 1, 1, SN_EPS, L.m);
    repack(c, L, L.m, L.m, false, true, 1);
    r.lP[1] = d_forward_rows(c, fake, B, B, drop, L.m, c->slab_k);
    launch_bce(c->logits, 2 * B, B, k.ls, 0.f, c->probs, c->dlogit, k.mt, 0, L.m, c->gscale);
    d_backward_pass(c, L, fake, B, fake, B, drop, true, false, BceSpec{B, 0.f, 0.f, nullptr, 0}, r.lP[1], B, c->sn_g[1]);
    repack(c, L, L.m, L.m, false, true, 0);
    d_backward_pass(c, L, c->real_stage, B, c->real_stage, B, drop, true, false, BceSpec{B, k.ls, k.ls, nullptr, 0}, r.lP[0], 0, c->sn_g[0]);
    SnTable t = c->snt;
    t.slot[0] = 0; t.slot[1] = 1;
    launch_sn_combine(t, c->sn_g[0], c->sn_g[1], c->st.d_grads, c->d_total, 2, L.m);
}

static void phase_d_grads(const siggan_ctx* c, Lanes& L, const PhaseKey& k, PhaseResult& r) {
    r.early_ar = 0;
    if (c->sn) return phase_d_grads_sn(c, L, k, r);
    const int B = k.B;
    const bool drop = c->cfg.dropout > 0.f;
    const bool nolane = k.pre_real == 2 && !k.d_dirty && (!drop || k.dreal_noise2);
    const float* xreal = c->real_stage;
    int P_real = k.lP0;
    if (nolane) {
        repack(c, L, L.m, L.m, k.g_dirty != 0, false);
        xreal = k.staged_src;
    } else {
    L.fork(L.a);
    repack(c, L, L.m, L.a, k.g_dirty != 0, k.d_dirty != 0);
    if (k.pre_real)
        L.note(hipMemcpyAsync(c->real_stage, k.staged_src, (size_t)B * c->S * c->S * sizeof(float), hipMemcpyDeviceToDevice, L.a));
    if (drop && !(k.pre_real == 2 && k.dreal_noise2))
        make_noise(c, k.has_masks ? c->mask_stage : nullptr, B, k.pre_real == 2 ? 1 : 0, 2, L.a);
    if (k.pre_real != 2) r.lP[0] = P_real = d_forward_rows(c, c->real_stage, 0, B, drop, L.a, c->slab_k2, true);
// ... 157 lines not shown

static int enqueue_phase(siggan_ctx* c, const PhaseKey& k, hipStream_t u, PhaseResult& r) {
    if (c->refused) return lane_check(c);
    const bool overlap = (c->mode & SIGGAN_MODE_OVERLAP) != 0;
    const bool graph = (c->mode & SIGGAN_MODE_GRAPH) != 0 && g_prof == nullptr;
    if (graph && c->comm && k.phase >= 2) return fail(SIGGAN_E_STATE, "SIGGAN_MODE_GRAPH is not available with a communicator");
    if (graph && c->sn) return fail(SIGGAN_E_STATE, "SIGGAN_MODE_GRAPH is not available with spectral normalisation");
    if (!graph) {
        const bool ext = overlap && g_prof == nullptr;
        Lanes L(c, u, overlap ? c->s_a : u, overlap ? c->s_b : u, ext);
        r = run_phase_body(c, L, k);
        LAUNCHCHK();
        return lane_check(c);
    }
    hipGraphExec_t exec = nullptr;
    for (auto& e : c->graphs)
        if (e.key == k) { exec = e.exec; r = e.res; break; }
    if (!exec) {
        Lanes L(c, c->s_m, overlap ? c->s_a : c->s_m, overlap ? c->s_b : c->s_m, false);
        hipGraph_t g = nullptr;
        HIPCHK(hipStreamBeginCapture(c->s_m, hipStreamCaptureModeRelaxed));
        r = run_phase_body(c, L, k);
        hipError_t e1 = hipStreamEndCapture(c->s_m, &g);
        if (e1 != hipSuccess || !g) return fail(SIGGAN_E_HIP, "stream capture failed: %s", hipGetErrorString(e1));
        if (c->refused) { (void)hipGraphDestroy(g); return lane_check(c); }
        hipError_t e2 = hipGraphInstantiate(&exec, g, nullptr, nullptr, 0);
        (void)hipGraphDestroy(g);
        if (e2 != hipSuccess) return fail(SIGGAN_E_HIP, "hipGraphInstantiate: %s", hipGetErrorString(e2));
        if (c->graphs.size() >= 64) { (void)hipGraphExecDestroy(c->graphs.front().exec); c->graphs.erase(c->graphs.begin()); }
        c->graphs.push_back(CachedPhase{k, exec, r});
    }
    hipEvent_t e_in = c->ev_bridge[0], e_out = c->ev_bridge[1];
    HIPCHK(hipEventRecord(e_in, u));
    HIPCHK(hipStreamWaitEvent(c->s_m, e_in, 0));
    HIPCHK(hipGraphLaunch(exec, c->s_m));
    HIPCHK(hipEventRecord(e_out, c->s_m));
    HIPCHK(hipStreamWaitEvent(u, e_out, 0));
    return SIGGAN_OK;
}
static int run_phase(siggan_ctx* c, const PhaseKey& k, hipStream_t u) {
    PhaseResult r;
    const int rc = enqueue_phase(c, k, u, r);
    Carried& cs = c->cs;
    auto put = [](auto& field, int v) { if (v >= 0) field = v; };
    put(cs.early_ar, r.early_ar); put(cs.dreal_joined, r.dreal_joined); put(cs.dreal_noise2, r.dreal_noise2);
    put(cs.gfwd_joined, r.gfwd_joined); put(cs.g_r0, r.g_r0); put(cs.ga_last_B, r.ga_last_B);
    put(cs.lP[0], r.lP[0]); put(cs.lP[1], r.lP[1]);
    return rc;
}

static PhaseKey make_key(siggan_ctx* c, int phase, int B, bool has_z, bool has_masks, const siggan_hyper* hp,
                         float* metrics_dev) {
    PhaseKey k; memset(&k, 0, sizeof k);
    k.phase = phase; k.B = B; k.has_z = has_z; k.has_masks = has_masks;
    k.mt = metrics_dev ? metrics_dev : c->metrics;
    if (phase <= 1) { k.g_dirty = c->g_dirty; k.d_dirty = c->d_dirty; k.ls = hp->label_smoothing; }
    else {
        k.lr = hp->lr; k.beta1 = hp->beta1; k.beta2 = hp->beta2; k.eps = hp->eps;
        k.clip = hp->clip_max_norm > 0.f ? hp->clip_max_norm : 0.f;
        k.gs = hp->grad_scale > 0.f ? hp->grad_scale : 1.0f;
    }
    return k;
}

static int finish_metrics(siggan_ctx* c, float* metrics_dev, float* metrics_host, hipStream_t s) {
    if (metrics_host) {
        HIPCHK(hipMemcpyAsync(metrics_host, metrics_dev ? metrics_dev : c->metrics, SIGGAN_M_COUNT * sizeof(float),
                              hipMemcpyDeviceToHost, s));
        HIPCHK(hipStreamSynchronize(s));
    }
    return SIGGAN_OK;
}

extern "C" int siggan_set_step_variant(siggan_ctx* c, int32_t variant) {
    if (!c) return fail(SIGGAN_E_INVALID, "null context");
    if (variant != SIGGAN_STEP_TRAINER && variant != SIGGAN_STEP_ABLATION) return fail(SIGGAN_E_INVALID, "unknown step variant %d", variant);
    if (c->cs.g_fwd_pending || c->cs.pending) return fail(SIGGAN_E_STATE, "a step is in flight");
    c->variant = variant;
    return SIGGAN_OK;
}

extern "C" int siggan_set_mode(siggan_ctx* c, int32_t mode) {
    if (!c) return fail(SIGGAN_E_INVALID, "null context");
    c->mode = mode;
    return SIGGAN_OK;
}

extern "C" int siggan_g_forward(siggan_ctx* c, const float* z_dev, int32_t batch, int32_t training, float* images_dev,
                                void* stream) {
    ENTER(c);
    int rc = check_call(c, batch);
    if (rc) return rc;
    if (training && (rc = check_bn_batch(c, batch))) return rc;
    if (!z_dev || !images_dev) return fail(SIGGAN_E_INVALID, "null tensor");
    hipStream_t s = (hipStream_t)stream;
    if ((rc = settle(c, s))) return rc;
    Lanes L(c, s);
    repack(c, L, s, s, c->g_dirty, !c->sn && c->d_dirty);
    c->g_dirty = false; if (!c->sn) c->d_dirty = false;
    c->cs.ga_last_B = g_forward_pass(c, z_dev, batch, training != 0, images_dev, s);
    if (training) c->g_dirty = true;
    LAUNCHCHK();
    return lane_check(c);
}

extern "C" int siggan_g_generate_u8(siggan_ctx* c, const float* z_dev, int32_t batch, uint8_t* u8_dev, float* images_dev,
                                    int32_t* stats_dev, float threshold, void* stream) {
    ENTER(c);
    int rc = check_call(c, batch);
    if (rc) return rc;
    if (!z_dev || !u8_dev) return fail(SIGGAN_E_INVALID, "null tensor");
    if (reinterpret_cast<uintptr_t>(u8_dev) & 3) return fail(SIGGAN_E_INVALID, "u8_dev must be 4-byte aligned");
    if (stats_dev && !isfinite(threshold)) return fail(SIGGAN_E_INVALID, "threshold must be finite");
    hipStream_t s = (hipStream_t)stream;
    if ((rc = settle(c, s))) return rc;
    Lanes L(c, s);
    repack(c, L, s, s, c->g_dirty, !c->sn && c->d_dirty);
    c->g_dirty = false; if (!c->sn) c->d_dirty = false;
    c->cs.ga_last_B = g_forward_pass(c, z_dev, batch, false, images_dev, s, nullptr, nullptr, 0, nullptr, nullptr, u8_dev, stats_dev, threshold);
    LAUNCHCHK();
    return lane_check(c);
}

extern "C" int siggan_d_forward(siggan_ctx* c, const float* x_dev, int32_t batch, int32_t training, const float* masks_dev,
                                float* probs_dev, float* features_dev, void* stream) {
    ENTER(c);
    int rc = check_call(c, batch);
    if (rc) return rc;
    if (!x_dev || (!probs_dev && !features_dev)) return fail(SIGGAN_E_INVALID, "null tensor");
    hipStream_t s = (hipStream_t)stream;
    invalidate(c, INV_ROWS);
    if ((rc = settle(c, s))) return rc;
    Lanes L(c, s);
    if (c->sn) launch_sn_sigma(c->snt, training != 0, 2, SN_EPS, s);
    repack(c, L, s, s, c->g_dirty, c->sn || c->d_dirty, 2);
    c->g_dirty = c->d_dirty = false;
    const bool drop = training != 0 && c->cfg.dropout > 0.f;
    if (drop) { if (!masks_dev) launch_tick(c->dev, s); make_noise(c, masks_dev, batch, 0, 1, s); }
    c->cs.lP[0] = d_forward_rows(c, x_dev, 0, batch, drop, s, c->slab_k);
    if (probs_dev) launch_bce(c->logits, batch, batch, 0.f, 0.f, probs_dev, nullptr, nullptr, 0, s);
    if (features_dev) launch_cls_features(c->dt, c->d_a[c->Ld], features_dev, batch, c->dC[c->Ld], s);
    LAUNCHCHK();
    return lane_check(c);
}

static int d_grads_common(siggan_ctx* c, const float* real_dev, int32_t batch, const float* z_dev, const float* masks_dev,
                          const siggan_hyper* hp, float* metrics_dev, void* stream, bool spec_g, const float* zg_dev,
                          bool apply_follows = false) {
    ENTER(c);
    Carried& cs = c->cs;
    int rc = check_call(c, batch);
    if (rc) return rc;
    if ((rc = check_hyper(hp))) return rc;
    if (!real_dev && cs.staged_B != batch)
        return fail(SIGGAN_E_INVALID, "null real batch (and no batch of %d images staged by siggan_stage_real)", batch);
    if (!c->st.d_grads) return fail(SIGGAN_E_STATE, "gradient arena was not bound");
    if (cs.g_fwd_pending) return fail(SIGGAN_E_STATE, "siggan_step_begin must be followed by siggan_g_grads before the next D step");
    if (spec_g && ((c->mode & SIGGAN_MODE_OVERLAP) == 0 || (c->mode & SIGGAN_MODE_GRAPH) != 0 || g_prof != nullptr)) spec_g = false;
    const bool abl = c->variant == SIGGAN_STEP_ABLATION;
    if (c->sn && !abl) spec_g = false;
    if (batch == 1 && !abl) spec_g = false;
    if (abl) {
        if ((rc = check_bn_batch(c, batch))) return rc;
        if (zg_dev) return fail(SIGGAN_E_INVALID, "the ablation step has one latent batch per iteration: pass it as z_dev");
        zg_dev = z_dev; z_dev = nullptr; spec_g = true;
    }
// ... 252 lines not shown
    ENTER(c);
    if (!c->comm) return SIGGAN_OK;
    HIPCHK(hipDeviceSynchronize());
    NCCLCHK(rccl()->CommDestroy(c->comm));
    c->comm = nullptr; c->comm_rank = 0; c->comm_world = 1; c->comm_err = 0;
    invalidate(c, INV_COMM);
    return SIGGAN_OK;
}
extern "C" int32_t siggan_comm_world(const siggan_ctx* c) { return c ? c->comm_world : -1; }
extern "C" int siggan_comm_broadcast(siggan_ctx* c, void* buf_dev, int64_t bytes, int32_t root, void* stream) {
    ENTER(c);
    if (!buf_dev || bytes < 1 || root < 0 || root >= c->comm_world) return fail(SIGGAN_E_INVALID, "bad argument");
    if (!c->comm) return SIGGAN_OK;
    NCCLCHK(rccl()->Broadcast(buf_dev, buf_dev, (size_t)bytes, NCCL_CHAR, root, c->comm, (hipStream_t)stream));
    return SIGGAN_OK;
}

extern "C" int siggan_device_info(int32_t device, int32_t* compute_units, int32_t* clock_khz, int64_t* hbm_bytes) {
    if (!compute_units || !clock_khz || !hbm_bytes) return fail(SIGGAN_E_INVALID, "null argument");
    hipDeviceProp_t p;
    HIPCHK(hipGetDeviceProperties(&p, device));
    *compute_units = p.multiProcessorCount; *clock_khz = p.clockRate; *hbm_bytes = (int64_t)p.totalGlobalMem;
    return SIGGAN_OK;
}

static Prof g_prof_store;
extern "C" int siggan_prof_enable(siggan_ctx* c, int32_t on) {
    if (!c) return fail(SIGGAN_E_INVALID, "null context");
    DevGuard dg_(c->cfg.device); HIPCHK(dg_.err);
    HIPCHK(hipDeviceSynchronize());
    g_prof_store.clear();
    g_prof = on ? &g_prof_store : nullptr;
    return SIGGAN_OK;
}
extern "C" int32_t siggan_prof_slots(void) { return Prof::NID - 1; }
extern "C" int siggan_prof_read(siggan_ctx* c, int32_t idx, char* name, int32_t name_cap, int64_t* launches, double* ms,
                                double* flops, double* bytes) {
    if (!c || !name || !launches || !ms || !flops || !bytes || idx < 0 || idx >= Prof::NID - 1) return fail(SIGGAN_E_INVALID, "bad argument");
    DevGuard dg_(c->cfg.device); HIPCHK(dg_.err);
    HIPCHK(hipDeviceSynchronize());
    snprintf(name, name_cap, "%s", Prof::name(idx));
    *launches = 0; *ms = 0.0; *flops = 0.0; *bytes = 0.0;
    for (auto& r : g_prof_store.recs) {
        if (r.id != idx) continue;
        float t = 0.f;
        HIPCHK(hipEventElapsedTime(&t, r.e0, r.e1));
        *launches += 1; *ms += t; *flops += r.flops; *bytes += r.bytes;
    }
    return SIGGAN_OK;
}

extern "C" int siggan_prof_launch(siggan_ctx* c, int64_t idx, int32_t* fields, int32_t n, int64_t* count) {
    if (!c || !count || (n > 0 && !fields)) return fail(SIGGAN_E_INVALID, "bad argument");
    *count = (int64_t)g_prof_store.recs.size();
    if (n <= 0) return SIGGAN_OK;
    if (idx < 0 || idx >= *count) return fail(SIGGAN_E_INVALID, "launch %lld of %lld", (long long)idx, (long long)*count);
    const Prof::Rec& r = g_prof_store.recs[(size_t)idx];
    const int32_t v[7] = {r.id, r.form, r.epi_req, r.epi, r.M, r.Ci, r.Co};
    for (int i = 0; i < n && i < 7; ++i) fields[i] = v[i];
    return SIGGAN_OK;
}

extern "C" int siggan_debug_tensor(siggan_ctx* c, const char* name, int32_t idx, float* out_dev, int64_t n, void* stream) {
    if (!c || !name || !out_dev || n < 1) return fail(SIGGAN_E_INVALID, "bad argument");
    const void* src = nullptr; int64_t capv = 0;
    const void** ptr = &src; int64_t* cap = &capv;
    bool typed = true;
    const int64_t Bm = c->Bm, Bd = 2 * Bm, SS = (int64_t)c->S * c->S;
    auto gsz = [&](int l) { const int64_t H = 4 << l; return Bm * H * H * c->gC[l]; };
    auto dsz = [&](int l) { const int64_t H = c->S >> l; return Bd * H * H * c->dC[l]; };
    const bool gl = idx >= 0 && idx <= c->Lg, dl = idx >= 1 && idx <= c->Ld;
    if (!strcmp(name, "g_y") && gl) { *ptr = c->g_y[idx]; *cap = gsz(idx); }
    else if (!strcmp(name, "g_a") && gl) { *ptr = c->g_a[idx]; *cap = gsz(idx); }
    else if (!strcmp(name, "g_da") && gl) { *ptr = c->g_da[idx]; *cap = gsz(idx); }
    else if (!strcmp(name, "d_a") && dl) { *ptr = c->d_a[idx]; *cap = dsz(idx); }
    else if (!strcmp(name, "d_dv") && dl) { *ptr = c->d_dv[idx]; *cap = dsz(idx); }
    else if (!strcmp(name, "d_a_g") && dl) {
        const int64_t H = c->S >> idx, off = (int64_t)c->cs.g_r0 * H * H * c->dC[idx];
        *ptr = c->d_a[idx] + (size_t)off * c->es; *cap = dsz(idx) - off;
    }
    else if (!strcmp(name, "z")) { *ptr = c->z; *cap = Bm * c->latent; typed = false; }
    else if (!strcmp(name, "z_g")) { *ptr = c->z_g; *cap = Bm * c->latent; typed = false; }
    else if (!strcmp(name, "img")) { *ptr = c->img; *cap = Bm * SS; typed = false; }
    else if (!strcmp(name, "dpre")) { *ptr = c->dpre; *cap = Bm * SS; typed = false; }
    else if (!strcmp(name, "logits")) { *ptr = c->logits; *cap = Bd; typed = false; }
    else if (!strcmp(name, "probs")) { *ptr = c->probs; *cap = Bd; typed = false; }
    else if (!strcmp(name, "dlogit")) { *ptr = c->dlogit; *cap = Bd; typed = false; }
    else if (!strcmp(name, "d_noise") && dl) { *ptr = c->d_noise[idx]; *cap = Bd * c->dC[idx]; typed = false; }
    else if (!strcmp(name, "rode") || !strcmp(name, "pre_real") || !strcmp(name, "ride_late")) {
        if (n != 1) return fail(SIGGAN_E_INVALID, "debug scalar %s holds 1 float, %lld asked", name, (long long)n);
        DevGuard dg_(c->cfg.device); HIPCHK(dg_.err);
        HIPCHK(hipStreamSynchronize((hipStream_t)stream));
        const float v = !strcmp(name, "rode") ? (float)c->cs.g_rode : !strcmp(name, "pre_real") ? (float)c->cs.g_pre_real
                                                                                               : (float)__atomic_load_n(c->ride_late, __ATOMIC_ACQUIRE);
        HIPCHK(hipMemcpy(out_dev, &v, sizeof v, hipMemcpyHostToDevice));
        return SIGGAN_OK;
    }
    else return fail(SIGGAN_E_INVALID, "unknown debug tensor %s[%d]", name, idx);
    if (n > capv) return fail(SIGGAN_E_INVALID, "debug tensor %s[%d] holds %lld floats, %lld asked", name, idx, (long long)capv, (long long)n);
    DevGuard dg_(c->cfg.device); HIPCHK(dg_.err);
    if (!strcmp(name, "g_a") && idx == c->Lg && c->cs.ga_last_B) {
        const int64_t H = c->S;
        HIPCHK(hipDeviceSynchronize());
        launch_bn_relu(c->dt, c->g_y[idx], c->g_a[idx], (int64_t)c->cs.ga_last_B * H * H, c->gC[idx], c->g_bn[idx], c->cfg.g_leaky_slope,
                       (hipStream_t)stream);
        LAUNCHCHK();
    }
    if (typed && c->dt != DT_F32) { launch_to_f32(c->dt, src, out_dev, n, (hipStream_t)stream); LAUNCHCHK(); }
    else HIPCHK(hipMemcpyAsync(out_dev, src, (size_t)n * sizeof(float), hipMemcpyDeviceToDevice, (hipStream_t)stream));
    return SIGGAN_OK;
}

extern "C" int siggan_augment_batch(int32_t device, const uint8_t* cache_dev, int64_t n_images, const int32_t* index_dev,
                                    const int32_t* params_dev, const int16_t* tables_dev, const float* lut_dev, float* out_dev,
                                    int32_t batch, int32_t size, int32_t augment, int32_t fill, void* stream) {
    if (!cache_dev || !index_dev || !lut_dev || !out_dev) return fail(SIGGAN_E_INVALID, "null tensor");
    if (augment && (!params_dev || !tables_dev)) return fail(SIGGAN_E_INVALID, "augment needs params and tables");
    if (batch < 1 || n_images < 1 || size < 1 || size > 1024) return fail(SIGGAN_E_INVALID, "bad batch / cache / image size");
    if (fill < 0 || fill > 255) return fail(SIGGAN_E_INVALID, "fill must be a byte value");
    DevGuard dg_(device); HIPCHK(dg_.err);
    launch_augment(cache_dev, n_images, index_dev, params_dev, tables_dev, lut_dev, out_dev, batch, size, augment != 0, fill, (hipStream_t)stream);
    LAUNCHCHK();
    return SIGGAN_OK;
}

extern "C" int siggan_image_stats(int32_t device, const float* x_dev, int32_t batch, int64_t pixels, float threshold,
                                  int32_t* stats_dev, void* stream) {
    if (!x_dev || !stats_dev) return fail(SIGGAN_E_INVALID, "null tensor");
    if (batch < 1 || pixels < 1) return fail(SIGGAN_E_INVALID, "bad batch / pixel count");
    if (!isfinite(threshold)) return fail(SIGGAN_E_INVALID, "threshold must be finite");
    if (reinterpret_cast<uintptr_t>(x_dev) & 3) return fail(SIGGAN_E_INVALID, "x_dev must be 4-byte aligned");
    if ((int64_t)batch * image_stats_chunks(pixels) > INT32_MAX) return fail(SIGGAN_E_INVALID, "batch too large for one launch");
    DevGuard dg_(device); HIPCHK(dg_.err);
    launch_image_stats(x_dev, batch, pixels, threshold, stats_dev, (hipStream_t)stream);
    LAUNCHCHK();
    return SIGGAN_OK;
}

extern "C" int siggan_op_randn(siggan_ctx* c, float* out_dev, int64_t n, void* stream) {
    if (!c || !out_dev || n < 1) return fail(SIGGAN_E_INVALID, "bad argument");
    DevGuard dg_(c->cfg.device); HIPCHK(dg_.err);
    hipStream_t s = (hipStream_t)stream;
    launch_tick(c->dev, s);
    launch_randn(out_dev, n, c->dev, 3, s);
    LAUNCHCHK();
    return SIGGAN_OK;
}
```

### signature-gan_amd/engine.py

```python
import ctypes as C

import torch

from . import _lib, layout


def _ptr(t):
    return C.c_void_p(t.data_ptr()) if t is not None else C.c_void_p(0)


def _f32(t, device, what):
    if t is None:
        return None
    if t.device != device:
        raise ValueError(f"{what} must live on {device}, got {t.device}")
    if t.dtype != torch.float32:
        raise ValueError(f"{what} must be float32, got {t.dtype}")
    return t.contiguous()


class Engine:

    def __init__(self, latent_dim=100, image_size=64, max_batch=64, device="cuda:0", seed=0,
                 dropout=0.25, leaky_slope=0.2, image_channels=1, dtype="f32", f16_grad_scale=0.0, spectral_norm=False,
# ... 54 lines not shown
                    self.sn_spans[key[:-len("weight")]] = (uo, rows, vo, cols)
                    uo, vo = uo + rows, vo + cols
            assert uo == self.lib.siggan_sn_count(h, 0) and vo == self.lib.siggan_sn_count(h, 1)
            self.d_sn_u, self.d_sn_v = z(uo), z(vo)
            gen = torch.Generator().manual_seed(self._seed & 0x7FFFFFFF)
            for base, (u0, rows, v0, cols) in self.sn_spans.items():
                self.d_sn_u[u0:u0 + rows] = torch.nn.functional.normalize(torch.randn(rows, generator=gen), dim=0, eps=1e-12).to(dev)
                self.d_sn_v[v0:v0 + cols] = torch.nn.functional.normalize(torch.randn(cols, generator=gen), dim=0, eps=1e-12).to(dev)
        self._bind()
        self.d_chans = list(layout.D_CHAIN[image_size])

    def _create_context(self):
        cfg = _lib.Config(self.device.index, self.latent_dim, self.image_size, 1, self.max_batch,
                          self.dropout, self.leaky_slope, self._seed, _lib.DTYPES[self.dtype], self.f16_grad_scale,
                          int(self.spectral_norm), self.g_slope)
        h = C.c_void_p()
        with torch.cuda.device(self.device):
            _lib.check(self.lib.siggan_create(C.byref(cfg), C.byref(h)))
        self._h = h

    def _bind(self):
        st = _lib.Storage(*[t.data_ptr() for t in (
            self.g_params, self.g_grads, self.g_exp_avg, self.g_exp_avg_sq, self.g_adam_steps, self.g_bn_mean,
            self.g_bn_var, self.g_bn_batches, self.d_params, self.d_grads, self.d_exp_avg, self.d_exp_avg_sq,
            self.d_adam_steps)] + [t.data_ptr() if t is not None else 0 for t in (self.d_sn_u, self.d_sn_v)])
        _lib.check(self.lib.siggan_bind(self._h, C.byref(st)))
        self._staged = None

    def ensure_batch(self, batch):
        if batch <= self.max_batch:
            return
        if self._comm is not None:
            raise RuntimeError(f"batch {batch} exceeds max_batch {self.max_batch}: a context that holds a communicator "
                               "cannot be re-created on one rank alone; size max_batch for the largest batch up front")
        torch.cuda.synchronize(self.device)
        seed, offset = self.rng_state()
        self.lib.siggan_destroy(self._h)
        self._h = None
        self._staged = None
        self.max_batch = 1 << (int(batch) - 1).bit_length()
        self._create_context()
        self._bind()
        if self._mode != 2:
            _lib.check(self.lib.siggan_set_mode(self._h, self._mode))
        self.seed(seed, offset)

    def views(self, which, arena="params"):
        spans = self.g_spans if which == "g" else self.d_spans
        flat = getattr(self, f"{which}_{arena}")
        return {k: flat[o:o + n].view(shape) for k, (o, n, shape) in spans.items()}

    def sn_views(self):
        out = {}
        for base, (u0, rows, v0, cols) in self.sn_spans.items():
            out[base + "weight_u"] = self.d_sn_u[u0:u0 + rows]
            out[base + "weight_v"] = self.d_sn_v[v0:v0 + cols]
        return out

    def bn_views(self):
        out = {}
        for i, (k, (o, n, shape)) in enumerate(self.bn_spans.items()):
            out[k] = self.g_bn_mean[o:o + n]
            out[k.replace("running_mean", "running_var")] = self.g_bn_var[o:o + n]
            out[k.replace("running_mean", "num_batches_tracked")] = self.g_bn_batches[i]
        return out

    def init_reference(self, seed=0):
        gen = torch.Generator().manual_seed(int(seed))
        for which in ("g", "d"):
            for k, v in self.views(which).items():
                if k.endswith("bias"):
                    v.zero_()
                else:
                    mean = 1.0 if ".1.weight" in k else 0.0
                    v.copy_(torch.empty(v.shape).normal_(mean, 0.02, generator=gen))
            for a in ("grads", "exp_avg", "exp_avg_sq", "adam_steps"):
                getattr(self, f"{which}_{a}").zero_()
        self.g_bn_mean.zero_(); self.g_bn_var.fill_(1.0); self.g_bn_batches.zero_()
        self.params_changed()

    def params_changed(self):
        _lib.check(self.lib.siggan_params_changed(self._h))

    def set_mode(self, graph=False, overlap=True):
        self._mode = (1 if graph else 0) | (2 if overlap else 0)
        _lib.check(self.lib.siggan_set_mode(self._h, self._mode))

    def set_step_variant(self, variant="trainer"):
        v = {"trainer": 0, "ablation": 1}[variant]
        _lib.check(self.lib.siggan_set_step_variant(self._h, v))
        self.step_variant = variant

    def ablation_step(self, real, z=None, masks=None, lr_d=2e-4, lr_g=2e-4, beta1=0.5, beta2=0.999, eps=1e-8,
                      label_smoothing=0.9, sync=True):
        if getattr(self, "step_variant", "trainer") != "ablation":
            raise RuntimeError("call set_step_variant('ablation') first")
        self.d_compute_grads(real, z, masks, label_smoothing, mask_passes=3)
        dm = self.d_apply(lr_d, beta1, beta2, eps, None, 1.0, sync)
        self.g_compute_grads(real.shape[0], label_smoothing=label_smoothing)
        gm = self.g_apply(lr_g, beta1, beta2, eps, None, 1.0, sync)
        if sync:
            dm.update(gm)
        return dm

    def seed(self, seed, offset=0):
        self._seed = int(seed)
        _lib.check(self.lib.siggan_seed(self._h, int(seed), int(offset)))

    def rng_state(self):
        s, o = C.c_uint64(), C.c_uint64()
        _lib.check(self.lib.siggan_rng_state(self._h, C.byref(s), C.byref(o)))
        return int(s.value), int(o.value)

    @staticmethod
    def comm_unique_id():
        buf = C.create_string_buffer(128)
        _lib.check(_lib.load().siggan_comm_unique_id(buf))
        return buf.raw

    def comm_init(self, rank, world, unique_id):
        if len(unique_id) != 128:
            raise ValueError("unique_id must be the 128 bytes of Engine.comm_unique_id()")
        self._comm_id = C.create_string_buffer(bytes(unique_id), 128)
        with torch.cuda.device(self.device):
            _lib.check(self.lib.siggan_comm_init(self._h, int(rank), int(world), self._comm_id))
        self._comm = (int(rank), int(world), bytes(unique_id))

    def comm_destroy(self):
        _lib.check(self.lib.siggan_comm_destroy(self._h))
        self._comm = None

    @property
    def comm_world(self):
        return int(self.lib.siggan_comm_world(self._h))

    def comm_broadcast(self, tensor, root=0):
        if tensor.device != self.device or not tensor.is_contiguous():
            raise ValueError("comm_broadcast needs a contiguous tensor on the engine's device")
        _lib.check(self.lib.siggan_comm_broadcast(self._h, _ptr(tensor), tensor.numel() * tensor.element_size(), int(root),
                                                  self._stream()))

    def _stream(self):
        return C.c_void_p(torch.cuda.current_stream(self.device).cuda_stream)

    def _hyper(self, lr, beta1, beta2, eps=1e-8, label_smoothing=0.9, clip=None, grad_scale=1.0):
        return _lib.Hyper(lr, beta1, beta2, eps, label_smoothing, clip if clip else 0.0, grad_scale)

    def _check_batch(self, b):
        if b < 1:
            raise ValueError(f"batch must be >= 1, got {b}")
        self.ensure_batch(b)

    def g_forward(self, z, training=False, out=None):
        z = _f32(z, self.device, "z")
        if z.dim() != 2 or z.shape[1] != self.latent_dim:
            raise ValueError(f"z must be (B, {self.latent_dim}), got {tuple(z.shape)}")
        b = z.shape[0]
        self._check_batch(b)
        if out is None:
            out = torch.empty(b, 1, self.image_size, self.image_size, dtype=torch.float32, device=self.device)
        _lib.check(self.lib.siggan_g_forward(self._h, _ptr(z), b, int(training), _ptr(out), self._stream()))
        return out

    def g_generate_u8(self, z, threshold=None, want_f32=False):
        b = 1
        if z is not None:
            z = _f32(z, self.device, "z")
            if z.dim() != 2 or z.shape[1] != self.latent_dim:
# ... 229 lines not shown
```

Baseline: 45190 images/s.

## Fuse final BN-backward apply into last generator input-gradient conv and alternate wgrad lanes

Adds a k_gconv_tail kernel that recomputes the final-layer activation gradient and BN backward in shared memory, then runs the 4x4 stride-2 input-gradient GEMM with the BN-backward statistics epilogue in the same kernel. This removes a separate launch and a global round-trip of the last-layer gradient. The BN reduction is split out into launch_final_fin. Generator weight-gradient kernels now alternate between two side streams with separate slabs, so adjacent layers' wgrads can overlap, at the cost of an extra slab allocation in f32. The fused path is the default in f32, and a new mode bit restores the unfused path.

Result: slower. 44580 images/s (-1.4%).

```diff
diff --git a/include/siggan.h b/include/siggan.h
--- a/include/siggan.h
+++ b/include/siggan.h
@@ -78,6 +78,7 @@
 int siggan_rng_state(siggan_ctx *ctx, uint64_t *seed, uint64_t *offset);
 #define SIGGAN_MODE_GRAPH 1
 #define SIGGAN_MODE_OVERLAP 2
+#define SIGGAN_MODE_UNFUSED_TAIL 4
 int siggan_set_mode(siggan_ctx *ctx, int32_t mode);
 
 enum { SIGGAN_STEP_TRAINER = 0, SIGGAN_STEP_ABLATION = 1 };
diff --git a/signature-gan_amd/csrc/final_bwd.h b/signature-gan_amd/csrc/final_bwd.h
--- /dev/null
+++ b/signature-gan_amd/csrc/final_bwd.h
@@ -0,0 +1,41 @@
+#pragma once
+#include "act.h"
+
+namespace siggan {
+
+typedef f32x4 f4v;
+
+template <int RY>
+__device__ __forceinline__ f4v final_dact(const float (&d)[RY + 2][3], const f4v (&w)[9], int r) {
+    f4v acc = {0.f, 0.f, 0.f, 0.f};
+#pragma unroll
+    for (int kh = 0; kh < 3; ++kh)
+#pragma unroll
+        for (int kw = 0; kw < 3; ++kw) {
+            const float g = d[r + 2 - kh][2 - kw];
+            const f4v ww = w[kh * 3 + kw];
+            acc.x = fmaf(g, ww.x, acc.x); acc.y = fmaf(g, ww.y, acc.y); acc.z = fmaf(g, ww.z, acc.z); acc.w = fmaf(g, ww.w, acc.w);
+        }
+    return acc;
+}
+
+struct FinalBnTab { f4v sc, sf, mu, rs, c1, c2; };
+__device__ __forceinline__ FinalBnTab final_bn_tab(const float* __restrict__ bn, int c4) {
+    constexpr int C = 32;
+    FinalBnTab t;
+    t.sc = *reinterpret_cast<const f4v*>(bn + c4 * 4); t.sf = *reinterpret_cast<const f4v*>(bn + C + c4 * 4);
+    t.mu = *reinterpret_cast<const f4v*>(bn + 2 * C + c4 * 4); t.rs = *reinterpret_cast<const f4v*>(bn + 3 * C + c4 * 4);
+    t.c1 = *reinterpret_cast<const f4v*>(bn + 4 * C + c4 * 4); t.c2 = *reinterpret_cast<const f4v*>(bn + 5 * C + c4 * 4);
+    return t;
+}
+template <bool LK>
+__device__ __forceinline__ f4v final_bn_bwd_apply4(const f4v g, const f4v v, const FinalBnTab& t, float gs) {
+    f4v o;
+    o.x = t.sc.x * (g_dact<LK>(fmaf(v.x, t.sc.x, t.sf.x), g.x, gs) - t.c1.x - (v.x - t.mu.x) * t.rs.x * t.c2.x);
+    o.y = t.sc.y * (g_dact<LK>(fmaf(v.y, t.sc.y, t.sf.y), g.y, gs) - t.c1.y - (v.y - t.mu.y) * t.rs.y * t.c2.y);
+    o.z = t.sc.z * (g_dact<LK>(fmaf(v.z, t.sc.z, t.sf.z), g.z, gs) - t.c1.z - (v.z - t.mu.z) * t.rs.z * t.c2.z);
+    o.w = t.sc.w * (g_dact<LK>(fmaf(v.w, t.sc.w, t.sf.w), g.w, gs) - t.c1.w - (v.w - t.mu.w) * t.rs.w * t.c2.w);
+    return o;
+}
+
+}
diff --git a/signature-gan_amd/csrc/gconv.h b/signature-gan_amd/csrc/gconv.h
--- a/signature-gan_amd/csrc/gconv.h
+++ b/signature-gan_amd/csrc/gconv.h
@@ -85,7 +85,7 @@
         int id; double flops, bytes; hipEvent_t e0, e1;
         int form, epi_req, epi, M, Ci, Co;
     };
-    static constexpr int NID = 8;
+    static constexpr int NID = 9;
     std::vector<Rec> recs;
     static const char* name(int id);
     void begin(int id, double flops, double bytes, hipStream_t st);
@@ -95,6 +95,15 @@
 extern Prof* g_prof;
 
 int launch_gconv(const GConvArgs& a, hipStream_t st);
+struct GTailArgs {
+    const float* dpre;
+    const float* wfin_t;
+    const float* y;
+    const float* bn;
+    float* dy;
+    int kper;
+};
+int launch_gconv_tail(const GConvArgs& a, const GTailArgs& t, hipStream_t st, hipEvent_t done);
 void launch_gconv16(int cfg, const GConvArgs& a, dim3 grid, hipStream_t st, hipEvent_t e0, hipEvent_t e1, int kq = 1);
 void launch_wgrad16(bool small, const WgradArgs& a, dim3 grid, hipStream_t st, hipEvent_t e0, hipEvent_t e1);
 int launch_wgrad(WgradArgs a, int max_splits, hipStream_t st);
diff --git a/signature-gan_amd/csrc/gconv.hip b/signature-gan_amd/csrc/gconv.hip
--- a/signature-gan_amd/csrc/gconv.hip
+++ b/signature-gan_amd/csrc/gconv.hip
@@ -1,4 +1,5 @@
 #include "gconv.h"
+#include "final_bwd.h"
 #include <hip/hip_ext.h>
 
 namespace siggan {
@@ -434,6 +435,161 @@
     for (int q = 0; q < (BM * 4 * BN / 4) / 256; ++q) dst[q * 256 + tid] = src[q * 256 + tid];
 }
 
+template <int S, bool LK>
+__global__ __launch_bounds__(256) void k_gconv_tail(const GConvArgs a, const GTailArgs t) {
+    constexpr int C = 32, BM = 128, BN = 32, LD = BK + 4, LP = C + 4, LDT = BN + 4;
+    constexpr int Wr = S / 2, R = BM / Wr, PR = 2 * R + 2, PC = S + 2;
+    constexpr int DR = PR + 2, DW = S + 2;
+    constexpr int NQ = PR * S / 32;
+    static_assert(BM * LDT + 4 * 256 * 8 <= PR * PC * LP, "output tile and statistics rows must fit the patch");
+    __shared__ __attribute__((aligned(16))) float smem[PR * PC * LP + 2 * BN * LD + DR * DW];
+    float* const sP = smem;
+    float* const sB = smem + PR * PC * LP;
+    float* const sD = sB + 2 * BN * LD;
+    const int tid = threadIdx.x, lane = tid & 63, wave = tid >> 6;
+    const int li = lane & 31, lh = lane >> 5;
+    const int bid = xcd_remap(blockIdx.x, gridDim.x), m0 = bid * BM;
+    const int n_img = m0 / (Wr * Wr), rh0 = (m0 / Wr) % Wr;
+    const int y0 = 2 * rh0 - 1;
+
+    const int kc = tid & 7, rloc = tid >> 3;
+    const float* const w_row = static_cast<const float*>(a.wp) + (size_t)rloc * (16 * C) + kc * 4;
+    f32x4 rb;
+    int l_tap = 0;
+    auto load_tile = [&]() __attribute__((always_inline)) { rb = *reinterpret_cast<const f32x4*>(w_row + l_tap * C); ++l_tap; };
+    auto store_tile = [&](int buf) __attribute__((always_inline)) {
+        *reinterpret_cast<f32x4*>(sB + (buf * BN + rloc) * LD + kc * 4) = rb;
+    };
+    load_tile();
+    store_tile(0);
+    load_tile();
+
+    {
+        const int c4 = tid & 7, xi = tid >> 3;
+        const float* const yimg = t.y + (size_t)n_img * S * S * C + c4 * 4;
+        f4v yv[NQ];
+#pragma unroll
+        for (int q = 0; q < NQ; ++q) {
+            const int i = xi + 32 * q, pr = i / S, x = i % S;
+            const int yy = y0 + pr, yc = yy < 0 ? 0 : (yy > S - 1 ? S - 1 : yy);
+            yv[q] = *reinterpret_cast<const f4v*>(yimg + ((size_t)yc * S + x) * C);
+        }
+        for (int i = tid; i < DR * DW; i += 256) {
+            const int r = i / DW, k = i - r * DW;
+            const int yy = y0 - 1 + r, xx = k - 1;
+            const int yc = yy < 0 ? 0 : (yy > S - 1 ? S - 1 : yy), xc = xx < 0 ? 0 : (xx > S - 1 ? S - 1 : xx);
+            const float q = t.dpre[((size_t)n_img * S + yc) * S + xc];
+            sD[i] = (yy == yc && xx == xc) ? q : 0.f;
+        }
+        f4v w[9];
+#pragma unroll
+        for (int k = 0; k < 9; ++k) w[k] = *reinterpret_cast<const f4v*>(t.wfin_t + k * 32 + c4 * 4);
+        const FinalBnTab tb = final_bn_tab(t.bn, c4);
+        if (tid < 2 * PR * 8)
+            *reinterpret_cast<f4v*>(sP + ((tid >> 4) * PC + ((tid >> 3) & 1) * (PC - 1)) * LP + c4 * 4) = f4v{0.f, 0.f, 0.f, 0.f};
+        __syncthreads();
+        float* const dyimg = t.dy + (size_t)n_img * S * S * C + c4 * 4;
+#pragma unroll
+        for (int q = 0; q < NQ; ++q) {
+            const int i = xi + 32 * q, pr = i / S, x = i % S;
+            const int yy = y0 + pr;
+            f4v o = {0.f, 0.f, 0.f, 0.f};
+            if ((unsigned)yy < (unsigned)S) {
+                float d[3][3];
+#pragma unroll
+                for (int r = 0; r < 3; ++r)
+#pragma unroll
+                    for (int k = 0; k < 3; ++k) d[r][k] = sD[(pr + r) * DW + x + k];
+                o = final_bn_bwd_apply4<LK>(final_dact<1>(d, w, 0), yv[q], tb, a.gslope);
+                if (pr >= 1 && pr <= PR - 2) *reinterpret_cast<f4v*>(dyimg + ((size_t)yy * S + x) * C) = o;
+            }
+            *reinterpret_cast<f4v*>(sP + (pr * PC + x + 1) * LP + c4 * 4) = o;
+        }
+    }
+    __syncthreads();
+
+    const int ml = wave * 32 + li;
+    const float* const pP = sP + ((2 * (ml / Wr)) * PC + 2 * (ml % Wr)) * LP + 4 * lh;
+    f32x16 acc, tot;
+#pragma unroll
+    for (int r = 0; r < 16; ++r) { acc[r] = 0.f; tot[r] = 0.f; }
+    const bool split = t.kper < 16;
+    int fold = t.kper;
+    for (int tap = 0; tap < 16; ++tap) {
+        const int buf = tap & 1;
+        const float* const pA = pP + ((tap >> 2) * PC + (tap & 3)) * LP;
+        const float* const pB = sB + (buf * BN + li) * LD + 4 * lh;
+        f32x4 fa[2], fb[2];
+        fa[0] = *reinterpret_cast<const f32x4*>(pA);
+        fb[0] = *reinterpret_cast<const f32x4*>(pB);
+#pragma unroll
+        for (int c = 0; c < BK / 8; ++c) {
+            const int cur = c & 1, nxt = cur ^ 1;
+            if (c + 1 < BK / 8) {
+                fa[nxt] = *reinterpret_cast<const f32x4*>(pA + 8 * (c + 1));
+                fb[nxt] = *reinterpret_cast<const f32x4*>(pB + 8 * (c + 1));
+            }
+            __builtin_amdgcn_sched_barrier(0);
+#pragma unroll
+            for (int u = 0; u < 4; ++u) acc = __builtin_amdgcn_mfma_f32_32x32x2f32(fa[cur][u], fb[cur][u], acc, 0, 0, 0);
+            if (c == 0 && tap + 1 < 16) store_tile(buf ^ 1);
+            if (c == 1 && tap + 2 < 16) load_tile();
+        }
+        __syncthreads();
+        if (split && (tap + 1 == fold || tap == 15)) {
+            if (tap + 1 == t.kper) tot = acc; else tot += acc;
+#pragma unroll
+            for (int r = 0; r < 16; ++r) acc[r] = 0.f;
+            fold += t.kper;
+        }
+    }
+    if (split) acc = tot;
+
+    float* const sT = smem;
+    float* const sS = smem + BM * LDT;
+#pragma unroll
+    for (int r = 0; r < 16; ++r) sT[(wave * 32 + (r & 3) + 8 * (r >> 2) + 4 * lh) * LDT + li] = acc[r];
+    __syncthreads();
+    constexpr int C4 = BN / 4, RPP = 256 / C4;
+    const int c4 = tid % C4, r0 = tid / C4, co = c4 * 4;
+    const BnBwdParams bq = bn_bwd_params(a.bnp, BN, co);
+    float* const outp = static_cast<float*>(a.out);
+    const float* const aref = static_cast<const float*>(a.aref);
+    f32x4 st0 = {0.f, 0.f, 0.f, 0.f}, st1 = st0;
+#pragma unroll
+    for (int p = 0; p < BM / RPP; ++p) {
+        const int row = r0 + RPP * p;
+        const size_t o = (size_t)(m0 + row) * BN + co;
+        const f32x4 v = *reinterpret_cast<const f32x4*>(sT + row * LDT + c4 * 4);
+        if (split) { st0 = f32x4{0.f, 0.f, 0.f, 0.f}; st1 = st0; }
+        bn_bwd_stat_terms<float, LK>(v, *reinterpret_cast<const f32x4*>(aref + o), bq, a.gslope, st0, st1);
+        *reinterpret_cast<f32x4*>(outp + o) = v;
+        if (split) {
+            *reinterpret_cast<f32x4*>(sS + (size_t)(p * 256 + tid) * 8) = st0;
+            *reinterpret_cast<f32x4*>(sS + (size_t)(p * 256 + tid) * 8 + 4) = st1;
+        }
+    }
+    if (!split) {
+        *reinterpret_cast<f32x4*>(sS + (size_t)tid * 8) = st0;
+        *reinterpret_cast<f32x4*>(sS + (size_t)tid * 8 + 4) = st1;
+    }
+    __syncthreads();
+    const int nrow = split ? BM / RPP : 1;
+    if (r0 < nrow) {
+        const float* const sr = sS + (size_t)r0 * 256 * 8;
+        st0 = *reinterpret_cast<const f32x4*>(sr + (size_t)c4 * 8);
+        st1 = *reinterpret_cast<const f32x4*>(sr + (size_t)c4 * 8 + 4);
+#pragma unroll 4
+        for (int k = 1; k < RPP; ++k) {
+            st0 += *reinterpret_cast<const f32x4*>(sr + (size_t)(k * C4 + c4) * 8);
+            st1 += *reinterpret_cast<const f32x4*>(sr + (size_t)(k * C4 + c4) * 8 + 4);
+        }
+        const size_t prow = (size_t)bid * nrow + r0;
+        *reinterpret_cast<f32x4*>(a.stat0 + prow * BN + co) = st0;
+        *reinterpret_cast<f32x4*>(a.stat1 + prow * BN + co) = st1;
+    }
+}
+
 template <class T, bool LK>
 __global__ __launch_bounds__(256) void k_splitk_epilogue(const GConvArgs a, int nsplit, int64_t total4) {
     const int64_t i = (int64_t)blockIdx.x * 256 + threadIdx.x;
@@ -515,7 +671,7 @@
 
 const char* Prof::name(int id) {
     static const char* n[NID] = {"k_gconv<128,128>", "k_gconv<128,64>", "k_gconv<64,64>", "k_gconv<128,32>",
-                                 "k_wgrad<64,64>", "k_gconv_up4", "k_wgrad<32,128>", "?"};
+                                 "k_wgrad<64,64>", "k_gconv_up4", "k_wgrad<32,128>", "k_gconv_tail", "?"};
     return n[id < 0 || id >= NID ? NID - 1 : id];
 }
 void Prof::begin(int id, double flops, double bytes, hipStream_t) {
@@ -582,6 +738,19 @@
     return rows;
 }
 
+static int split_count(const GConvArgs& a, int nblk, int nk) {
+    int ns = 1;
+    if (a.slab && nblk < 384) {
+        ns = (512 + nblk - 1) / nblk;
+        if (ns > nk / 4) ns = nk / 4;
+        if (ns > 8) ns = 8;
+        const int64_t out_floats = (int64_t)a.B * a.Ho * a.Wo * a.Co;
+        if (ns > 1 && (int64_t)ns * out_floats > a.slab_floats) ns = (int)(a.slab_floats / out_floats);
+        if (ns < 1) ns = 1;
+    }
+    return ns;
+}
+
 int launch_gconv(const GConvArgs& a_in, hipStream_t st) {
     GConvArgs a = a_in;
     if (a.epi == EPI_BN_BWD_STATS && (a.stat0 == nullptr || a.stat_cap <= 0)) return -1;
@@ -589,17 +758,8 @@
     auto blocks = [&](int bm, int bn) { return ((a.M + bm - 1) / bm) * (a.Co / bn) * ncls; };
     const int nk = (a.form == 0 ? 16 : 4) * (a.Ci / BK);
     auto splits = [&](int nblk) {
-        int ns = 1;
-        if (a.slab && nblk < 384) {
-            ns = (512 + nblk - 1) / nblk;
-            if (ns > nk / 4) ns = nk / 4;
-            if (ns > 8) ns = 8;
-            const int64_t out_floats = (int64_t)a.B * a.Ho * a.Wo * a.Co;
-            if (ns > 1 && (int64_t)ns * out_floats > a.slab_floats) ns = (int)(a.slab_floats / out_floats);
-            if (ns < 1) ns = 1;
-        }
         a.slab_stride = (size_t)a.B * a.Ho * a.Wo * a.Co;
-        return ns;
+        return split_count(a, nblk, nk);
     };
     if (a.Co >= 64) {
         if (a.Co >= 128 && blocks(128, 128) >= 512) return launch_cfg<128, 128, 2, 2, 32, 1>(a, st, 0, 1);
@@ -628,6 +788,33 @@
     }
     const int ns = splits(blocks(128, 32));
     return launch_cfg<128, 32, 4, 1, 32, 1>(a, st, 3, ns);
+}
+
+int launch_gconv_tail(const GConvArgs& a_in, const GTailArgs& t_in, hipStream_t st, hipEvent_t done) {
+    GConvArgs a = a_in;
+    GTailArgs t = t_in;
+    const int S = a.Hi, Hr = S / 2;
+    if (a.dt != DT_F32 || a.form != 0 || a.epi != EPI_BN_BWD_STATS || a.Ci != 32 || a.Co != 32 || (S != 64 && S != 128) || a.Wi != S ||
+        a.Ho != Hr || a.Wo != Hr || a.M != a.B * Hr * Hr || a.stat0 == nullptr)
+        return -1;
+    const int tiles = a.M / 128;
+    const int ns = split_count(a, tiles, 16);
+    const int rows = ns > 1 ? a.M / 32 : tiles;
+    if ((int64_t)2 * rows * a.Co > a.stat_cap) return -1;
+    a.stat1 = a.stat0 + (size_t)rows * a.Co;
+    t.kper = (16 + ns - 1) / ns;
+    if (g_prof) {
+        g_prof->begin(7, 2.0 * a.M * a.Co * (double)(16 * a.Ci), gconv_bytes(a), st);
+        g_prof->shape(a, a_in.epi);
+    }
+    hipEvent_t e0 = g_prof ? g_prof->recs.back().e0 : nullptr, e1 = g_prof ? g_prof->recs.back().e1 : done;
+    const dim3 grid(tiles);
+    SIGGAN_GS_SWITCH(a.gslope, LK, {
+        if (S == 64) hipExtLaunchKernelGGL((k_gconv_tail<64, LK>), grid, dim3(256), 0, st, e0, e1, 0, a, t);
+        else hipExtLaunchKernelGGL((k_gconv_tail<128, LK>), grid, dim3(256), 0, st, e0, e1, 0, a, t);
+    });
+    if (g_prof && done) (void)hipEventRecord(done, st);
+    return rows;
 }
 
 template <int BM, int BN, int WM, int WN>
diff --git a/signature-gan_amd/csrc/ops.h b/signature-gan_amd/csrc/ops.h
--- a/signature-gan_amd/csrc/ops.h
+++ b/signature-gan_amd/csrc/ops.h
@@ -70,9 +70,10 @@
                       int32_t* stats = nullptr, float thr = 0.f);
 void launch_final_bwd_reduce(int dt, const float* dpre, const float* Wt, const void* y, int B, int S, int C, const float* bn,
                              float* partial, float* partial_w, float gslope, hipStream_t s);
-void launch_final_bn_bwd_apply(int dt, const float* dpre, const float* Wt, const void* y, void* dy, int B, int S, int C, float* bn,
-                               const float* partial, const float* partial_w, float* dW, float* db, float* dgamma, float* dbeta,
-                               float gslope, hipStream_t s, hipEvent_t done = nullptr);
+void launch_final_fin(int B, int S, int C, float* bn, const float* partial, const float* partial_w, float* dW, float* db,
+                      float* dgamma, float* dbeta, hipStream_t s);
+void launch_final_bn_bwd_apply(int dt, const float* dpre, const float* Wt, const void* y, void* dy, int B, int S, int C,
+                               const float* bn, float gslope, hipStream_t s, hipEvent_t done = nullptr);
 
 void launch_conv1_fwd(int dt, const float* x0, int n0, const float* x1, const float* W, const float* b,
                       const float* noise, float slope, void* out, int B, int S, int C, hipStream_t s);
diff --git a/signature-gan_amd/csrc/ops.hip b/signature-gan_amd/csrc/ops.hip
--- a/signature-gan_amd/csrc/ops.hip
+++ b/signature-gan_amd/csrc/ops.hip
@@ -1,4 +1,5 @@
 #include "ops.h"
+#include "final_bwd.h"
 #include "../../include/siggan.h"
 #include "rng.h"
 
@@ -541,7 +542,6 @@
                                                 B, K, C0));
 }
 
-typedef f32x4 f4v;
 __device__ __forceinline__ f4v ldg4(const float* p) { return *reinterpret_cast<const f4v*>(p); }
 __device__ __forceinline__ int clampi(int v, int hi) { return v < 0 ? 0 : (v > hi ? hi : v); }
 
@@ -692,19 +692,6 @@
 #pragma unroll
         for (int k = 0; k < 3; ++k) d[r][k] = sp[r * 34 + xi + k];
 }
-template <int RY>
-__device__ __forceinline__ f4v final_dact(const float (&d)[RY + 2][3], const f4v (&w)[9], int r) {
-    f4v acc = {0.f, 0.f, 0.f, 0.f};
-#pragma unroll
-    for (int kh = 0; kh < 3; ++kh)
-#pragma unroll
-        for (int kw = 0; kw < 3; ++kw) {
-            const float g = d[r + 2 - kh][2 - kw];
-            const f4v ww = w[kh * 3 + kw];
-            acc.x = fmaf(g, ww.x, acc.x); acc.y = fmaf(g, ww.y, acc.y); acc.z = fmaf(g, ww.z, acc.z); acc.w = fmaf(g, ww.w, acc.w);
-        }
-    return acc;
-}
 
 template <class T, int RY, bool LK>
 __global__ __launch_bounds__(256) void k_final_bwd_reduce(const float* __restrict__ dpre, const float* __restrict__ Wt,
@@ -816,8 +803,7 @@
     f4v w[9];
 #pragma unroll
     for (int k = 0; k < 9; ++k) w[k] = ldg4(Wt + k * 32 + c4 * 4);
-    const f4v sc = ldg4(bn + c4 * 4), sf = ldg4(bn + C + c4 * 4), mu = ldg4(bn + 2 * C + c4 * 4), rs = ldg4(bn + 3 * C + c4 * 4);
-    const f4v c1 = ldg4(bn + 4 * C + c4 * 4), c2 = ldg4(bn + 5 * C + c4 * 4);
+    const FinalBnTab tb = final_bn_tab(bn, c4);
     __shared__ float sp[(RY + 2) * 34];
     const int xi = threadIdx.x >> 3;
     const float pe = dpre_patch_elem<RY>(dpre, t.n, t.y0, t.x - xi, S, threadIdx.x);
@@ -832,12 +818,7 @@
 #pragma unroll
     for (int r = 0; r < RY; ++r) {
         const f4v g = final_dact<RY>(d, w, r);
-        const f4v v = yv[r];
-        f4v o;
-        o.x = sc.x * (g_dact<LK>(fmaf(v.x, sc.x, sf.x), g.x, gs) - c1.x - (v.x - mu.x) * rs.x * c2.x);
-        o.y = sc.y * (g_dact<LK>(fmaf(v.y, sc.y, sf.y), g.y, gs) - c1.y - (v.y - mu.y) * rs.y * c2.y);
-        o.z = sc.z * (g_dact<LK>(fmaf(v.z, sc.z, sf.z), g.z, gs) - c1.z - (v.z - mu.z) * rs.z * c2.z);
-        o.w = sc.w * (g_dact<LK>(fmaf(v.w, sc.w, sf.w), g.w, gs) - c1.w - (v.w - mu.w) * rs.w * c2.w);
+        const f4v o = final_bn_bwd_apply4<LK>(g, yv[r], tb, gs);
         st4<T>(dy + o0 + (size_t)r * S * C, o);
     }
 }
@@ -882,14 +863,18 @@
     SIGGAN_GS_SWITCH(gslope, LK, SIGGAN_DT_SWITCH(dt, T, hipLaunchKernelGGL((k_final_bwd_reduce<T, FINAL_RY, LK>), dim3(nch), dim3(256), 0, s, dpre, Wt,
                                                                      (const T*)y, bn, p0, p1, partial_w, S, nstrips, gslope)));
 }
-void launch_final_bn_bwd_apply(int dt, const float* dpre, const float* Wt, const void* y, void* dy, int B, int S, int C, float* bn,
-                               const float* partial, const float* partial_w, float* dW, float* db, float* dgamma, float* dbeta,
-                               float gslope, hipStream_t s, hipEvent_t done) {
-    const int nstrips = B * (S / 4) * (S / 32), nch = final_reduce_rows(B, S);
+void launch_final_fin(int B, int S, int C, float* bn, const float* partial, const float* partial_w, float* dW, float* db,
+                      float* dgamma, float* dbeta, hipStream_t s) {
+    const int nch = final_reduce_rows(B, S);
     const float* p0 = partial; const float* p1 = partial + (size_t)nch * C;
     const int nbw = cdiv(C * 9 + 1, 64);
     hipLaunchKernelGGL(k_final_fin, dim3(nbw + cdiv(C, 32)), dim3(1024), 0, s, partial_w, nch, C * 9 + 1, dW, C * 9, db, nbw, p0, p1, nch,
                        (int64_t)B * S * S, C, bn, dgamma, dbeta);
+}
+void launch_final_bn_bwd_apply(int dt, const float* dpre, const float* Wt, const void* y, void* dy, int B, int S, int C,
+                               const float* bn, float gslope, hipStream_t s, hipEvent_t done) {
+    (void)C;
+    const int nstrips = B * (S / 4) * (S / 32);
     SIGGAN_GS_SWITCH(gslope, LK, SIGGAN_DT_SWITCH(dt, T, SIGGAN_LAUNCH_EV(done, (k_final_bnbwd_apply<T, LK>), dim3(nstrips), dim3(256), 0, s, dpre, Wt,
                                                                    (const T*)y, bn, (T*)dy, S, gslope)));
 }
diff --git a/signature-gan_amd/csrc/siggan.hip b/signature-gan_amd/csrc/siggan.hip
--- a/signature-gan_amd/csrc/siggan.hip
+++ b/signature-gan_amd/csrc/siggan.hip
@@ -359,7 +359,7 @@
         carve(&c->wcp, (int64_t)c->dC[c->Ld] * 16);
         carve(&c->slab, c->slab_floats);
         carve(&c->slab_k, c->slab_k_floats);
-        if (c->dt != DT_F32) carve(&c->slab_b, c->slab_floats); else if (pass == 1) c->slab_b = c->slab;
+        carve(&c->slab_b, c->slab_floats);
         carve(&c->slab_k2, c->slab_k_floats);
         if (c->dt != DT_F32) carve(&c->slab_k3, c->slab_k_floats); else if (pass == 1) c->slab_k3 = c->slab_k2;
         carve(&c->partial, PARTIAL_FLOATS);
@@ -866,23 +866,13 @@
 static void g_backward_pass(const siggan_ctx* c, Lanes& L, const float* z, int B) {
     const float gs = c->cfg.g_leaky_slope;
     const int Lg = c->Lg, S = c->S;
+    const bool tail = c->dt == DT_F32 && (c->mode & SIGGAN_MODE_UNFUSED_TAIL) == 0;
     int pre_rows = 0;
     for (int l = Lg; l >= 1; --l) {
         const int Hi = 4 << (l - 1), Ho = 2 * Hi, Ci = c->gC[l - 1], Co = c->gC[l];
         const int64_t R = (int64_t)B * Ho * Ho;
-        hipEvent_t const ef = L.fork_event(L.a);
-        if (l == Lg) {
-            launch_final_bwd_reduce(c->dt, c->dpre, c->wfin_t, c->g_y[l], B, S, Co, c->g_bn[l], c->partial, c->partial_b, gs, L.m);
-            launch_final_bn_bwd_apply(c->dt, c->dpre, c->wfin_t, c->g_y[l], c->g_da[l], B, S, Co, c->g_bn[l], c->partial, c->partial_b,
-                                      GG(c, gi_fin_w(c)), GG(c, gi_fin_b(c)), GG(c, gi_bn_w(l)), GG(c, gi_bn_b(l)), gs, L.m, ef);
-        } else
-            launch_bn_bwd(c->dt, c->g_da[l], c->g_y[l], R, Co, c->g_bn[l], c->partial, GG(c, gi_bn_w(l)), GG(c, gi_bn_b(l)), 0, gs, L.m, pre_rows, ef);
-        L.fork_after(L.a, ef);
-        WgradArgs w; memset(&w, 0, sizeof w); w.zeros = c->zeros; w.dt = c->dt;
-        w.S = c->g_a[l - 1]; w.L = c->g_da[l]; w.slab = c->slab; w.dw = GG(c, gi_up_w(l)); w.B = B; w.Cs = Ci; w.Cl = Co;
-        w.lgHs = ilog2i(Hi); w.lgWs = w.lgHs; w.lgCl = ilog2i(Co); w.K = B * Hi * Hi;
-        const int max_splits = (int)(c->slab_floats / ((int64_t)Ci * (16 * Co + 1)));
-        launch_wgrad(w, max_splits, L.a);
+        const bool lane_b = tail && ((Lg - l) & 1) != 0;
+        hipStream_t const lw = lane_b ? L.b : L.a;
         GConvArgs a = gconv_args(c);
         a.in = c->g_da[l]; a.wp = c->g_dn[l]; a.out = c->g_da[l - 1];
         a.B = B; a.Hi = Ho; a.Wi = Ho; a.Ci = Co; a.Co = Ci;
@@ -890,7 +880,28 @@
         if (l >= 2) {
             a.epi = EPI_BN_BWD_STATS; a.aref = c->g_y[l - 1]; a.bnp = c->g_bn[l - 1]; a.stat0 = c->partial; a.stat_cap = PARTIAL_FLOATS;
         }
-        pre_rows = launch_gconv(a, L.m);
+        hipEvent_t const ef = L.fork_event(lw);
+        int tail_rows = -1;
+        if (l == Lg) {
+            launch_final_bwd_reduce(c->dt, c->dpre, c->wfin_t, c->g_y[l], B, S, Co, c->g_bn[l], c->partial, c->partial_b, gs, L.m);
+            launch_final_fin(B, S, Co, c->g_bn[l], c->partial, c->partial_b, GG(c, gi_fin_w(c)), GG(c, gi_fin_b(c)), GG(c, gi_bn_w(l)),
+                             GG(c, gi_bn_b(l)), L.m);
+            if (tail) {
+                GTailArgs t; memset(&t, 0, sizeof t);
+                t.dpre = c->dpre; t.wfin_t = c->wfin_t; t.y = (const float*)c->g_y[l]; t.bn = c->g_bn[l]; t.dy = (float*)c->g_da[l];
+                tail_rows = launch_gconv_tail(a, t, L.m, ef);
+            }
+            if (tail_rows < 0)
+                launch_final_bn_bwd_apply(c->dt, c->dpre, c->wfin_t, c->g_y[l], c->g_da[l], B, S, Co, c->g_bn[l], gs, L.m, ef);
+        } else
+            launch_bn_bwd(c->dt, c->g_da[l], c->g_y[l], R, Co, c->g_bn[l], c->partial, GG(c, gi_bn_w(l)), GG(c, gi_bn_b(l)), 0, gs, L.m, pre_rows, ef);
+        L.fork_after(lw, ef);
+        WgradArgs w; memset(&w, 0, sizeof w); w.zeros = c->zeros; w.dt = c->dt;
+        w.S = c->g_a[l - 1]; w.L = c->g_da[l]; w.slab = lane_b ? c->slab_b : c->slab; w.dw = GG(c, gi_up_w(l)); w.B = B; w.Cs = Ci; w.Cl = Co;
+        w.lgHs = ilog2i(Hi); w.lgWs = w.lgHs; w.lgCl = ilog2i(Co); w.K = B * Hi * Hi;
+        const int max_splits = (int)(c->slab_floats / ((int64_t)Ci * (16 * Co + 1)));
+        launch_wgrad(w, max_splits, lw);
+        pre_rows = tail_rows >= 0 ? tail_rows : launch_gconv(a, L.m);
         if (pre_rows < 0) {
             L.refuse("the Generator's input-gradient GEMM was refused: its BatchNorm-backward sums had no carve (stat_cap)");
             pre_rows = 0;
@@ -902,6 +913,7 @@
                       c->gC[0], gs, L.m);
         launch_fc_wgrad(c->dt, c->g_da[0], z, GG(c, gi_fc_w()), GG(c, gi_fc_b()), B, c->latent, c->gC[0], L.m);
     }
+    if (tail) L.join(L.b);
     L.join(L.a);
 }
 
@@ -1225,6 +1237,7 @@
 
 extern "C" int siggan_set_mode(siggan_ctx* c, int32_t mode) {
     if (!c) return fail(SIGGAN_E_INVALID, "null context");
+    if (mode & ~(SIGGAN_MODE_GRAPH | SIGGAN_MODE_OVERLAP | SIGGAN_MODE_UNFUSED_TAIL)) return fail(SIGGAN_E_INVALID, "unknown mode bits %d", mode);
     c->mode = mode;
     return SIGGAN_OK;
 }
@@ -1643,6 +1656,7 @@
     else if (!strcmp(name, "z")) { *ptr = c->z; *cap = Bm * c->latent; typed = false; }
     else if (!strcmp(name, "z_g")) { *ptr = c->z_g; *cap = Bm * c->latent; typed = false; }
     else if (!strcmp(name, "img")) { *ptr = c->img; *cap = Bm * SS; typed = false; }
+    else if (!strcmp(name, "partial")) { *ptr = c->partial; *cap = PARTIAL_FLOATS; typed = false; }
     else if (!strcmp(name, "dpre")) { *ptr = c->dpre; *cap = Bm * SS; typed = false; }
     else if (!strcmp(name, "logits")) { *ptr = c->logits; *cap = Bd; typed = false; }
     else if (!strcmp(name, "probs")) { *ptr = c->probs; *cap = Bd; typed = false; }
diff --git a/signature-gan_amd/engine.py b/signature-gan_amd/engine.py
--- a/signature-gan_amd/engine.py
+++ b/signature-gan_amd/engine.py
@@ -160,8 +160,8 @@
     def params_changed(self):
         _lib.check(self.lib.siggan_params_changed(self._h))
 
-    def set_mode(self, graph=False, overlap=True):
-        self._mode = (1 if graph else 0) | (2 if overlap else 0)
+    def set_mode(self, graph=False, overlap=True, unfused_tail=False):
+        self._mode = (1 if graph else 0) | (2 if overlap else 0) | (4 if unfused_tail else 0)
         _lib.check(self.lib.siggan_set_mode(self._h, self._mode))
 
     def set_step_variant(self, variant="trainer"):
```
